# cbs228/sameold

Measured on AMD Instinct MI355X. Metric: Msamples/s demodulated (batched 22.05 kHz channels) + % HBM roofline, 1/8 GPU, higher is better.
Workload: dtype f32

## Files before the change

### include/same_rx.h

```cpp
#ifndef SAME_RX_H
#define SAME_RX_H

#include <stddef.h>
#include <stdint.h>

#ifdef __cplusplus
extern "C" {
#endif

#define SAME_RX_ABI_VERSION 2

enum {
    SAME_OK = 0,
    SAME_EINVAL = -1,
    SAME_EDCLEN = -2,
    SAME_EAGCLIMITS = -3,
    SAME_EEQORDER = -4,
    SAME_ENODEVICE = -5,
    SAME_EHIP = -6,
    SAME_EOVERFLOW = -7,
    SAME_ENOMEM = -8,
    SAME_ERATE = -9,
    SAME_EKERNEL = -10
};
// ... 54 lines not shown

#define SAME_EVENT_MAX_BYTES 288

typedef struct same_rx_event {
    uint32_t kind;
    uint32_t channel;
    uint64_t sample_counter;
    uint64_t symbol_count;
    uint32_t len;
    uint32_t aux;
    uint32_t aux2;
    uint32_t reserved;
    uint8_t bytes[SAME_EVENT_MAX_BYTES];
} same_rx_event;

enum { SAME_LAYOUT_TIME_MAJOR = 0, SAME_LAYOUT_CHANNEL_MAJOR = 1 };

enum {
    SAME_BATCH_LINK_ONLY = 1u << 0,
    SAME_BATCH_TRACE_SYMBOLS = 1u << 1,
    SAME_BATCH_GENERIC_KERNEL = 1u << 2,
    SAME_BATCH_TIME_PARALLEL = 1u << 3,
    SAME_BATCH_RELAXED = 1u << 4,
    SAME_BATCH_CALL_INVARIANT = 1u << 5,
    SAME_BATCH_MESSAGES_ONLY = 1u << 6
};
#define SAME_TP_EVENT_TOLERANCE_SYMBOLS 2

typedef struct same_batch same_batch;

int same_batch_new(const same_rx_builder *b, uint32_t n_channels, int device,
                   uint32_t flags, same_batch **out);
void same_batch_free(same_batch *rx);
int same_batch_reset(same_batch *rx);
int same_batch_reset_channels(same_batch *rx, const uint32_t *channels, size_t n);
uint64_t same_batch_channel_input_sample_counter(const same_batch *rx, uint32_t channel);
uint32_t same_batch_input_rate(const same_batch *rx);
uint32_t same_batch_n_channels(const same_batch *rx);
uint64_t same_batch_input_sample_counter(const same_batch *rx);
int same_batch_device(const same_batch *rx);

#define SAME_STREAM_OWN ((void *)(intptr_t)-1)
int same_batch_process_device(same_batch *rx, const float *d_x, size_t n_samples,
                              uint32_t layout, void *hip_stream);
int same_batch_set_call_window(same_batch *rx, uint32_t samples);
int same_batch_order_after(same_batch *rx, void *producer_stream);
int same_batch_process_device_i16(same_batch *rx, const int16_t *d_x, size_t n_samples,
                                  uint32_t layout, void *hip_stream);
int same_batch_process_host(same_batch *rx, const float *h_x, size_t n_samples, uint32_t layout);
int same_batch_process_host_i16(same_batch *rx, const int16_t *h_x, size_t n_samples, uint32_t layout);
int same_batch_process_device_ragged(same_batch *rx, const float *d_x, size_t n_rows, const uint32_t *counts,
                                     uint32_t layout, void *hip_stream);
int same_batch_process_device_ragged_i16(same_batch *rx, const int16_t *d_x, size_t n_rows, const uint32_t *counts,
                                         uint32_t layout, void *hip_stream);
int same_batch_process_host_ragged(same_batch *rx, const float *h_x, size_t n_rows, const uint32_t *counts, uint32_t layout);
int same_batch_process_host_ragged_i16(same_batch *rx, const int16_t *h_x, size_t n_rows, const uint32_t *counts,
                                       uint32_t layout);
int same_batch_flush(same_batch *rx);
int same_batch_sync(same_batch *rx);

int same_batch_poll_events(same_batch *rx, same_rx_event *out, size_t cap, size_t *n_out,
                           size_t *n_left);
size_t same_batch_pending_events(same_batch *rx);
int same_batch_peek_events(same_batch *rx, const same_rx_event **events, size_t *n);
int same_batch_drop_events(same_batch *rx, size_t n);
#define SAME_BURST_RECORD_BYTES 304
int same_batch_pack_bursts(same_batch *rx, uint32_t first_channel, uint8_t *out, size_t cap, size_t *n_records);

int same_batch_time_parallel_config(same_batch *rx, uint32_t max_chunks, uint32_t min_own_samples,
                                    uint32_t warmup_samples);
uint32_t same_batch_time_parallel_chunks(const same_batch *rx);
int same_batch_time_parallel_per_channel(const same_batch *rx);

typedef struct same_tp_plan_info {
    uint32_t channels, n_chunks, block_len, warmup_samples, whole_samples, scout_blocks;
    uint32_t sort_mode, lpt, pair_groups;
    uint32_t reserved;
    uint64_t in_samples;
    uint64_t counter0;
    uint64_t w_own_start, w_row0, w_nominal, w_perm, w_wg, w_wg2, w_perm2, w_total;
} same_tp_plan_info;
int same_batch_debug_tp_plan(same_batch *rx, same_tp_plan_info *info, float *energy, size_t energy_cap, uint32_t *geom,
                             size_t geom_cap, uint64_t *handover, size_t handover_cap, uint32_t *final_col, size_t final_col_cap);

int same_batch_transport_on_device(const same_batch *rx);

enum {
    SAME_AUDIO_FIRST = 1,
    SAME_AUDIO_END_MESSAGE = 2,
    SAME_AUDIO_END_FLUSH = 4,
    SAME_AUDIO_END_RESET = 8,
    SAME_AUDIO_TRUNCATED = 16
};
typedef struct same_audio_chunk {
    uint32_t channel, flags;
    uint64_t sample_counter;
    uint64_t n_samples;
    const float *samples;
} same_audio_chunk;
int same_batch_set_audio_capture(same_batch *rx, size_t samples_per_launch);
int same_batch_peek_audio(same_batch *rx, const same_audio_chunk **chunks, size_t *n);
int same_batch_drop_audio(same_batch *rx, size_t n);

typedef struct same_symbol_trace {
    uint64_t sample_counter;
    float zero, sym, err, samples_until_next_ted;
} same_symbol_trace;
int same_batch_read_trace(same_batch *rx, uint32_t channel, same_symbol_trace *out,
                          size_t cap, size_t *n_out);

int same_batch_last_kernel_ms(same_batch *rx, float *ms);
int same_batch_last_demod_kernel_ms(same_batch *rx, float *ms);
void same_batch_set_kernel_timing(same_batch *rx, int enable);
const char *same_batch_kernel_name(const same_batch *rx);

typedef struct same_rx same_rx;
int same_rx_build(const same_rx_builder *b, int device, same_rx **out);
void same_rx_free(same_rx *rx);
int same_rx_process(same_rx *rx, const float *x, size_t n, size_t *consumed, same_rx_event *ev);
int same_rx_flush(same_rx *rx, same_rx_event *msg);
int same_rx_reset(same_rx *rx);
uint32_t same_rx_input_rate(const same_rx *rx);
uint64_t same_rx_input_sample_counter(const same_rx *rx);

int same_synth_afsk_device(float *d_x, uint32_t n_channels, size_t n_samples,
                           uint32_t input_rate, uint64_t seed, float noise_sigma,
                           uint32_t flags, int device, void *hip_stream);
uint32_t same_synth_payload(uint64_t seed, uint32_t channel, uint8_t *out, uint32_t cap);
int same_synth_trials_device(float *d_x, uint32_t n_trials, uint32_t first_trial, size_t n_samples,
                             uint32_t input_rate, uint64_t seed, float ebn0_db_lo, float ebn0_db_step,
                             uint32_t n_grid, int device, void *hip_stream);

#ifdef __cplusplus
}
#endif
#endif
```

### sameold_amd/csrc/same_batch.cpp

```cpp
#include <hip/hip_runtime.h>

#include <algorithm>
#include <chrono>
#include <cstdio>
#include <cstdlib>
#include <cstring>
#include <deque>
#include <new>
#include <string>
#include <type_traits>
#include <utility>
#include <vector>

#include "../../include/same_rx.h"
#include "same_config.h"
#include "same_device.h"
#include "same_harvest.h"
#include "same_hipmem.h"
#include "same_launch.h"
#include "same_resets.h"
#include "same_tp_plan.h"
#include "same_transport.h"

using same::fail;
static_assert(sizeof(same::cap::Span) == same::kSpanBytes, "same_tp_plan.h sizes the span list");

namespace {

#define HIP_TRY(expr)                                                                     \
    do {                                                                                   \
        hipError_t _e = (expr);                                                            \
        if (_e != hipSuccess)                                                              \
            return fail(SAME_EHIP, "%s failed: %s (%s:%d)", #expr, hipGetErrorString(_e),  \
                        __FILE__, __LINE__);                                               \
    } while (0)

}

struct same_batch {
    same_rx_builder builder{};
    same::Params P{};
    same::State S{};
    int device = 0;
    uint32_t flags = 0;
    uint64_t counter = 0;
    hipStream_t own_stream = nullptr;
    hipStream_t last_stream = nullptr;
    same::DevBuf<float4> d_taps;
    same::DevBuf<void> d_state_blob;
    struct Slot {
        same::DevBuf<same::DevEvent> d_events;
        uint32_t event_cap() const { return (uint32_t)d_events.size(); }
        same::DevBuf<uint32_t> d_sort;
        same::PinnedBuf<uint32_t> h_sort;
        same::DevBuf<same::DevEvent> d_sorted;
        uint32_t sort_bins = 0;
        same::DevBuf<uint8_t> d_bursts;
        uint32_t burst_cap() const { return (uint32_t)(d_bursts.size() / same::kBurstCap); }
        same::DevBuf<uint32_t> d_counters;
        same::MappedBuf<uint32_t> h_counters;
        same::Event ev_start, ev_stop, ev_done, ev_planned;
        same::Event ev_k0, ev_k1;
        bool have_k = false;
        bool timed = false;
        same::PinnedBuf<void> h_events, h_bursts;
        bool in_flight = false;
        uint64_t seq = 0;
        uint64_t end_counter = 0;
        bool chunked = false;
        same::ChunkGeom geom{};
        uint32_t columns(uint32_t n_channels) const { return chunked ? geom.n_chunks * n_channels : n_channels; }
        uint64_t end_blocks = 0;
        same::DevBuf<uint64_t> d_handover;
        same::PinnedBuf<uint64_t> h_handover;
        bool per_channel = false;
        same::TpGeomWords words;
        same::DevBuf<uint32_t> d_geom;
        same::PinnedBuf<uint32_t> h_geom;
        same::TpPlan plan{};
        uint64_t plan_counter0 = 0;
        bool plan_sorted = false, plan_lpt = false, plan_pairs = false;
        same::CoherentBuf<uint32_t> h_reset;
        same::CoherentBuf<uint32_t> h_counts;
        same::PinnedBuf<uint64_t> h_wake_up;
        bool dev_transport = false;
        same::CoherentBuf<same::DevMessage> h_near;
        uint32_t near_cap() const { return (uint32_t)h_near.size(); }
        same::DevBuf<same::DevMessage> d_msgs;
        uint32_t msg_cap() const { return (uint32_t)d_msgs.size(); }
        same::PinnedBuf<void> h_msgs;
        bool captured = false;
        same::DevBuf<same::cap::Span> d_spans;
        uint32_t span_cap() const { return (uint32_t)d_spans.size(); }
        same::DevBuf<float> d_pool;
        same::DevBuf<same::cap::Cursors> d_cap_cur;
        same::MappedBuf<same::cap::Cursors> h_cap_cur;
        same::PinnedBuf<void> h_spans, h_pool;
    } slot[2];
    struct TimePar {
        bool enabled = false;
        same::TpConfig cfg;
        uint32_t cap_columns = 0;
        uint32_t carved_columns = 0;
        int carved_family = -1;
        same::Params Pv{};
        same::State Sv{};
        same::DevBuf<void> blob;
        same::DevBuf<void> blob_fresh;
        size_t fresh_bytes = 0;
        same::DevBuf<same::StateArrayDesc> d_desc_in, d_desc_out;
        uint32_t n_desc = 0;
        same::DevBuf<uint32_t> d_final_col;
        same::DevBuf<float> d_energy;
        same::DevBuf<float> d_hist;
        same::Event ev_plan_prev; bool plan_recorded = false;
        uint32_t last_chunks = 1;
        bool last_per_channel = false;
        same::Family family = same::Family::kPipe;
    } tp;
    uint64_t launch_seq = 0;
    hipStream_t copy_stream = nullptr;
    struct Windowed {
        bool on = false;
        uint32_t window = 0;
        uint32_t fill = 0;
        same::DevBuf<void> d_buf;
        same::Event ev_buf;
        hipStream_t buf_stream = nullptr; bool buf_used = false;
        same::Event ev_read[2];
        uint64_t n_reads = 0;
        hipStream_t read_stream = nullptr;
    } inv;
    hipStream_t plan_stream = nullptr;
    float last_ms = 0.0f;
    bool overflowed = false;
    std::string record_path;
    bool kernel_fault = false;
    same::Request want;
    same::Mode mode;
    same::Choice plain;
    same::Params Pfm{};
    same::Family last_family = same::Family::kGeneric;
    bool sym_launched = false;
    bool debug = false;
    same::DevBuf<void> d_stage, d_stage2;
    same::DevBuf<void> d_upload;
    same::DevBuf<void> d_zero;
    same::Event ev_order;
    bool timing = false;
    bool have_timing = false;
    float last_demod_ms = 0.0f;
    same::PinnedBuf<uint64_t> h_wake;
    bool wake_ordered = false;
    std::vector<uint32_t> ragged_by;
    bool messages_only = false;
    bool dev_transport = false;
    bool last_dev_transport = false;
    same::DevBuf<void> d_thot, d_tcold;
    same::ResetLedger resets;
    std::vector<uint32_t> reset_list, reset_now, reset_cols;
    same::EventLog events;
    same::Replay replay{resets, events};
    struct Audio {
        size_t per_launch = 0;
        same::DevBuf<same::cap::Rec> d_rec;
        uint64_t flush_at = UINT64_MAX;
        same::AudioLog log;
    } audio;
};

namespace {

struct Carver {
    size_t off = 0;
    template <typename T> size_t take(size_t n)
    {
        off = (off + 255) & ~size_t(255);
        size_t o = off;
        off += n * sizeof(T);
        return o;
    }
};

#define SAME_STATE_ARRAYS(X, P)                                                                            \
    X(dc_ff_ring, float, (P).dc_len) X(dc_fb_ring, float, (P).dc_len)                                        \
    X(dc_sum0, float, 1) X(dc_sum1, float, 1) X(agc_gain, float, 1)                                          \
    X(win_ring, float, (P).win_ring)                                                                         \
    X(ted_clock, uint32_t, 1) X(until_next_ted, float, 1)                                                    \
    X(ted_h0, float, 1) X(ted_h1, float, 1) X(ted_h2, float, 1)                                              \
    X(period_avg, float, 1) X(period_inst, float, 1)                                                         \
    X(sq_data, uint32_t, 1) X(sq_power, float, 1) X(sq_phist, uint32_t, 1)                                   \
    X(sq_fill, uint32_t, 1) X(sq_clock, int32_t, 1) X(sq_symbols, uint64_t, 1)                               \
    X(sq_hist, float, same::kSquelchHist)                                                                    \
    X(eq_ffc, float, (P).eq_nff) X(eq_fbc, float, (P).eq_nfb)                                                \
    X(eq_ffw, float, (P).eq_nff) X(eq_fbw, float, (P).eq_nfb)                                                \
    X(eq_word, uint32_t, 1) X(eq_count, uint32_t, 1)                                                         \
    X(eq_snap_ffc, float, (P).eq_nff) X(eq_snap_fbc, float, (P).eq_nfb)                                      \
// ... 297 lines not shown
    }
    return SAME_OK;
}

int harvest(same_batch *rx)
{
    same_batch::Slot *order[2] = {&rx->slot[0], &rx->slot[1]};
    if (order[0]->seq > order[1]->seq) std::swap(order[0], order[1]);
    for (same_batch::Slot *sl : order) {
        int rc = harvest_slot(rx, *sl);
        if (rc) return rc;
    }
    return SAME_OK;
}

int ensure_wide_state(same_batch *rx, uint32_t columns)
{
    same_batch::TimePar &tp = rx->tp;
    if (tp.carved_columns == columns && tp.carved_family == (int)tp.family) return SAME_OK;
    int rc = harvest(rx);
    if (rc) return rc;
    HIP_TRY(hipDeviceSynchronize());
    tp.Pv = same::wide_params(rx->P, columns, same::is_fastmath(tp.family), same::tp_more_than_one_round(columns));
    if (columns > tp.cap_columns) {
        tp.cap_columns = 0;
        HIP_TRY(tp.blob.reset());
        HIP_TRY(tp.blob_fresh.reset());
        const size_t bytes = carve_state(tp.Pv, nullptr, tp.Sv);
        HIP_TRY(tp.blob.ensure(bytes));
        HIP_TRY(hipMemset(tp.blob, 0, bytes));
        HIP_TRY(tp.blob_fresh.ensure(bytes));
        tp.cap_columns = columns;
    }
    const size_t blob_bytes = carve_state(tp.Pv, (char *)tp.blob.get(), tp.Sv);
    {
        same::State Sf{};
        carve_state(tp.Pv, (char *)tp.blob_fresh.get(), Sf);
        HIP_TRY(hipMemset(tp.blob_fresh, 0, blob_bytes));
        HIP_TRY(same::launch_init_state(tp.Pv, Sf, 0, nullptr, 0));
        HIP_TRY(hipDeviceSynchronize());
        tp.fresh_bytes = (size_t)(reinterpret_cast<char *>(tp.Sv.fr_msg) - static_cast<char *>(tp.blob.get()));
    }
    std::vector<same::StateArrayDesc> in, out;
    list_state_arrays(rx->P, rx->S, tp.Sv, in);
    list_state_arrays(rx->P, tp.Sv, rx->S, out);
    tp.n_desc = (uint32_t)in.size();
    HIP_TRY(tp.d_desc_in.ensure(in.size()));
    HIP_TRY(tp.d_desc_out.ensure(out.size()));
    HIP_TRY(tp.d_final_col.ensure(rx->P.n_channels));
    HIP_TRY(hipMemcpy(tp.d_desc_in, in.data(), in.size() * sizeof(same::StateArrayDesc), hipMemcpyHostToDevice));
    HIP_TRY(hipMemcpy(tp.d_desc_out, out.data(), out.size() * sizeof(same::StateArrayDesc), hipMemcpyHostToDevice));
    tp.carved_columns = columns;
    tp.carved_family = (int)tp.family;
    return SAME_OK;
}

struct Ragged {
    const uint32_t *counts = nullptr;
    uint32_t m = 0;
    uint32_t row_off = 0;
};

struct RaggedLaunch {
    uint32_t row0 = 0;
    size_t n_lock = 0;
};


int begin_launch(same_batch *rx, same_batch::Slot &sl, const same_batch::Slot &prev, hipStream_t stream)
{
    int rc = harvest_slot(rx, sl);
    if (rc) return rc;
    if (prev.in_flight && rx->last_stream != stream) HIP_TRY(hipStreamWaitEvent(stream, prev.ev_done, 0));
    return launch_pending_resets(rx, sl, stream);
}

int begin_timing(same_batch *rx, same_batch::Slot &sl, hipStream_t stream)
{
    sl.timed = rx->timing;
    if (sl.timed) HIP_TRY(hipEventRecord(sl.ev_start, stream));
    return SAME_OK;
}

int tp_start(same_batch *rx, same_batch::Slot &sl, uint32_t columns, const char *layout, hipStream_t stream, bool *sort_bins_empty)
{
    same_batch::TimePar &tp = rx->tp;
    const uint32_t C = rx->P.n_channels;
    *sort_bins_empty = false;
    if (tp.cfg.knob_prologue >= 0) {
        HIP_TRY(same::launch_tp_prologue(tp.blob, tp.blob_fresh, tp.fresh_bytes, sl.d_handover, sl.d_sort, columns, sl.d_counters, stream));
        *sort_bins_empty = sl.sort_bins == columns;
    } else {
        HIP_TRY(same::launch_counters(sl.d_counters, sl.h_counters.dev(), 0, stream));
        HIP_TRY(same::launch_init_state(tp.Pv, tp.Sv, 0, stream, C));
        HIP_TRY(same::launch_fill_u64(sl.d_handover, columns, same::kNoHandover, stream));
    }
    if (rx->debug) std::fprintf(stderr, "[same] time-parallel launch: %u columns (%s), start-up: %s\n", columns, layout,
                                tp.cfg.knob_prologue >= 0 ? "prologue kernel" : "separate launches");
    HIP_TRY(same::launch_copy_state_columns(tp.d_desc_in, tp.n_desc, C, columns, nullptr, C, stream));
    return SAME_OK;
}

template <typename SampleT>
int demod_tail(same_batch *rx, const same::Output &O, const SampleT *rows, size_t n, uint64_t counter0, hipStream_t stream)
{
    const hipError_t e = same::launch_demod(rx->P, rx->S, O, rx->d_taps, rows, (uint32_t)n, counter0, stream);
    if (e != hipSuccess) return fail(SAME_EHIP, "demod kernel launch failed: %s", hipGetErrorString(e));
    return SAME_OK;
}
int demod_tail_corner(same_batch *rx, const same::Output &O, const float *corner, size_t pitch, size_t r, uint64_t counter0, hipStream_t stream)
{
    const uint32_t C = rx->P.n_channels;
    HIP_TRY(rx->d_stage.ensure(r * C * sizeof(float)));
    HIP_TRY(rx->d_stage2.ensure(r * C * sizeof(float)));
    float *staged = static_cast<float *>(rx->d_stage.get()), *rows = static_cast<float *>(rx->d_stage2.get());
    HIP_TRY(hipMemcpy2DAsync(staged, r * sizeof(float), corner, pitch * sizeof(float), r * sizeof(float), C, hipMemcpyDeviceToDevice, stream));
    const hipError_t e = same::launch_transpose(staged, rows, C, (uint32_t)r, stream);
    if (e != hipSuccess) return fail(SAME_EHIP, "demod kernel launch failed: %s", hipGetErrorString(e));
    return demod_tail(rx, O, rows, r, counter0, stream);
}

int tp_plan_boundaries(same_batch *rx, same_batch::Slot &sl, const same::TpCut &cut, const same::TpNative &np, const float *d_x,
                       hipStream_t stream, same::PipeChunks &pc)
{
    same_batch::TimePar &tp = rx->tp;
    const same::TpGeomWords &w = np.words;
    same::TpPlan plan{};
    plan.channels = rx->P.n_channels; plan.n_chunks = cut.n_chunks; plan.block_len = cut.geom.block_len;
    plan.warmup_samples = np.warmup_samples; plan.whole_samples = np.whole_samples; plan.in_samples = np.in_samples;
    plan.scout_blocks = np.scout_blocks;
    sl.plan = plan; sl.plan_counter0 = rx->counter;
    sl.plan_sorted = np.sort_mode != 0; sl.plan_lpt = np.lpt; sl.plan_pairs = np.pair_groups;
    uint32_t *g = sl.d_geom;
    const bool side = same::tp_plan_beside(tp.cfg, stream == rx->own_stream);
    hipStream_t ps = side ? rx->plan_stream : stream;
    if (tp.plan_recorded) HIP_TRY(hipStreamWaitEvent(ps, tp.ev_plan_prev, 0));
    HIP_TRY(same::launch_tp_plan(d_x, plan, tp.d_energy, g + w.own_start, g + w.row0, g + w.nominal, g + w.perm, g + w.wg, np.sort_mode != 0, ps,
                                 np.lpt ? g + w.perm2 : nullptr, np.lpt ? g + w.wg2 : nullptr, np.pair_groups));
    HIP_TRY(tp.ev_plan_prev.ensure());
    HIP_TRY(hipEventRecord(tp.ev_plan_prev, ps));
    tp.plan_recorded = true;
    if (side) {
        HIP_TRY(hipEventRecord(sl.ev_planned, ps));
        HIP_TRY(hipStreamWaitEvent(stream, sl.ev_planned, 0));
    }
    pc.col_row0 = g + w.row0; pc.col_nominal = g + w.nominal;
    pc.wg_blocks = g + (np.lpt ? w.wg2 : w.wg); pc.col_perm = np.lpt ? g + w.perm2 : nullptr;
    pc.in_samples = np.in_samples; pc.whole_samples = np.whole_samples;
    pc.hist_scratch = np.need_hist ? tp.d_hist.get() : nullptr;
    return SAME_OK;
}

template <typename SampleT>
int launch_time_parallel(same_batch *rx, same_batch::Slot &sl, hipStream_t stream, const same::TpCut &cut, const same::TpNative *np,
                         const SampleT *x, size_t n_call, bool *sort_bins_empty)
{
    same_batch::TimePar &tp = rx->tp;
    const same::ChunkGeom &geom = cut.geom;
    const uint32_t C = rx->P.n_channels, columns = cut.n_chunks * C, fb = geom.block_len;
    const uint32_t total_blocks = (uint32_t)(n_call / fb);
    const size_t n_whole = (size_t)total_blocks * fb;
    tp.family = cut.choice.family;
    same::Output O{};
    int rc = ensure_wide_state(rx, columns);
    if (rc == SAME_OK) rc = ensure_output(rx, sl, same::tp_output_samples(np ? n_whole : n_call, cut.pc, fb), O, columns);
    if (rc) return rc;
    HIP_TRY(sl.d_handover.ensure(columns));
    HIP_TRY(sl.h_handover.ensure(columns));
    same::PipeChunks pc = cut.pc;
    pc.handover = sl.d_handover;
    if (np) {
        HIP_TRY(sl.d_geom.ensure(np->words.total));
        HIP_TRY(sl.h_geom.ensure(np->words.harvest));
        HIP_TRY(tp.d_energy.ensure(np->energy_floats));
        if (np->need_hist) HIP_TRY(tp.d_hist.ensure(np->hist_floats));
        sl.words = np->words;
    }
    rc = begin_timing(rx, sl, stream);
    if (rc) return rc;
    const float *xf = nullptr;
    if constexpr (std::is_same_v<SampleT, float>) xf = x;
    if (np && (rc = tp_plan_boundaries(rx, sl, cut, *np, xf, stream, pc)) != SAME_OK) return rc;
    rc = tp_start(rx, sl, columns, np ? "channel-major" : "time-major", stream, sort_bins_empty);
    if (rc) return rc;
    sl.have_k = np && sl.timed;
    if (sl.have_k) HIP_TRY(hipEventRecord(sl.ev_k0, stream));
    const hipError_t e = launch_family(tp.family, tp.Pv, tp.Sv, O, rx->d_taps, x, total_blocks, rx->counter, stream, pc);
    rx->last_family = tp.family;
    if (e != hipSuccess) return fail(SAME_EHIP, "time-parallel demod kernel launch failed: %s", hipGetErrorString(e));
    if (sl.have_k) HIP_TRY(hipEventRecord(sl.ev_k1, stream));
    if (np) HIP_TRY(same::launch_chunk_final_column_pc(sl.d_handover, sl.d_geom + np->words.own_start, C, geom.n_chunks, rx->counter, tp.d_final_col, stream));
    else HIP_TRY(same::launch_chunk_final_column(sl.d_handover, C, geom, tp.d_final_col, stream));
    HIP_TRY(same::launch_copy_state_columns(tp.d_desc_out, tp.n_desc, columns, C, tp.d_final_col, C, stream));
    if (n_whole < n_call) {
        rc = np ? demod_tail_corner(rx, O, xf + n_whole, n_call, n_call - n_whole, rx->counter + n_whole, stream)
                : demod_tail(rx, O, x + n_whole * C, n_call - n_whole, rx->counter + n_whole, stream);
        if (rc) return rc;
    }
    sl.chunked = true; sl.per_channel = np != nullptr;
    sl.geom = geom;
    sl.end_blocks = rx->counter + n_whole;
    tp.last_chunks = cut.n_chunks; tp.last_per_channel = sl.per_channel;
    return SAME_OK;
}

template <typename SampleT>
int end_launch(same_batch *rx, same_batch::Slot &sl, same_batch::Slot &prev, hipStream_t stream, const SampleT *rows, size_t n,
               bool sort_bins_empty, const RaggedLaunch *rl = nullptr)
{
    if (sl.timed) HIP_TRY(hipEventRecord(sl.ev_stop, stream));
    HIP_TRY(same::launch_event_sort(sl.d_events, sl.d_counters, sl.event_cap(), sl.sort_bins, sl.d_sort, sl.d_sort + sl.sort_bins,
                                    sl.d_sorted, stream, sort_bins_empty));
    sl.dev_transport = rx->dev_transport && !sl.chunked;
    rx->last_dev_transport = sl.dev_transport;
    if (sl.dev_transport) {
        same::TransportLaunch T{};
        T.n_channels = rx->P.n_channels; T.input_rate = rx->P.input_rate;
        T.first = sl.d_sort + sl.sort_bins; T.sorted = sl.d_sorted; T.counters = sl.d_counters;
        T.bursts = sl.d_bursts; T.burst_cap = sl.burst_cap();
        T.hot = rx->d_thot; T.cold = rx->d_tcold; T.wake_sample = rx->S.wake_sample;
        T.near = sl.h_near.dev(); T.near_cap = sl.near_cap();
        T.log = sl.d_msgs; T.log_cap = sl.msg_cap(); T.log_cursor = sl.d_counters + 3; T.overflow = sl.d_counters + 2;
        sl.captured = rx->audio.per_launch != 0;
        if (sl.captured) {
            same::cap::Launch &K = T.cap;
            const uint64_t fa = rx->audio.flush_at;
            K.start = rx->counter; K.n_rows = (uint32_t)n;
            K.flush_row = fa >= rx->counter + n ? same::cap::kNoFlush : (uint32_t)(fa > rx->counter ? fa - rx->counter : 0);
            K.rec = rx->audio.d_rec; K.spans = sl.d_spans; K.span_cap = sl.span_cap();
            K.n_spans = &sl.d_cap_cur->n_spans; K.pool_used = &sl.d_cap_cur->pool_used; K.pool_cap = rx->audio.per_launch;
            K.overflow = &sl.d_cap_cur->overflow;
        }
        if (rl && rl->n_lock < n)
            HIP_TRY(same::launch_transport_ragged(T, sl.h_counts.dev(), rl->row0, (uint32_t)n, stream));
        else
            HIP_TRY(same::launch_transport(T, stream));
        if (sl.captured) {
            const hipError_t e = same::launch_capture(sl.d_spans, sl.d_cap_cur, sl.span_cap(), sl.d_pool, rx->audio.per_launch, rows,
                                                      rx->P.n_channels, (uint32_t)n, sl.h_cap_cur.dev(), stream);
            if (e != hipSuccess) return fail(SAME_EHIP, "capture kernel launch failed: %s", hipGetErrorString(e));
        }
    }
    HIP_TRY(same::launch_counters(sl.d_counters, sl.h_counters.dev(), 1, stream));
    HIP_TRY(hipEventRecord(sl.ev_done, stream));
    sl.in_flight = true;
    sl.seq = ++rx->launch_seq;
    rx->last_stream = stream;
    if (rl) rx->resets.shift(rx->ragged_by.data(), rx->counter + n, (int)(&sl - rx->slot));
    rx->counter += n;
    sl.end_counter = rx->counter;
    return harvest_slot(rx, prev);
}

template <typename SampleT>
int process_time_major_launches(same_batch *rx, const SampleT *d_x, size_t n_samples, hipStream_t stream, const Ragged *rg = nullptr)
{
    const size_t kMaxChunk = same::max_launch_samples(rx->P.input_rate);
    size_t done = 0;
    while (done < n_samples) {
        const size_t n = std::min(kMaxChunk, n_samples - done);
        same_batch::Slot &sl = rx->slot[rx->launch_seq & 1];
        same_batch::Slot &prev = rx->slot[(rx->launch_seq & 1) ^ 1];
        int rc = begin_launch(rx, sl, prev, stream);
        if (rc) return rc;
        size_t n_lock = n;
        if (rg) {
            const size_t row0 = (size_t)rg->row_off + done;
            const uint32_t C = rx->P.n_channels;
            HIP_TRY(sl.h_counts.ensure(C));
            std::memcpy(sl.h_counts, rg->counts, (size_t)C * sizeof(uint32_t));
            rx->ragged_by.resize(C);
            n_lock = same::ragged_launch_split(rg->counts, C, rg->m, row0, n, rx->ragged_by.data());
        }
        const same::TpCut cut = rg ? same::TpCut{} : same::tp_uniform_cut(rx->P, rx->mode, rx->want, rx->tp.cfg, n, rx->counter);
        rx->tp.last_chunks = cut.n_chunks;
        sl.have_k = false;
// ... 649 lines not shown
    if (!rx || !n_out) return fail(SAME_EINVAL, "null argument");
    if (!rx->P.trace_cap) return fail(SAME_EINVAL, "batch was not created with SAME_BATCH_TRACE_SYMBOLS");
    if (channel >= rx->P.n_channels) return fail(SAME_EINVAL, "channel out of range");
    HIP_TRY(hipSetDevice(rx->device));
    int rc = harvest(rx);
    if (rc) return rc;
    uint32_t n = 0;
    HIP_TRY(hipMemcpy(&n, rx->S.trace_n + channel, sizeof(n), hipMemcpyDeviceToHost));
    n = std::min(n, rx->P.trace_cap);
    n = (uint32_t)std::min<size_t>(n, cap);
    std::vector<float> f((size_t)n * 4);
    std::vector<uint64_t> idx(n);
    if (n) {
        HIP_TRY(hipMemcpy(f.data(), rx->S.trace + (size_t)channel * rx->P.trace_cap * 4, f.size() * sizeof(float), hipMemcpyDeviceToHost));
        HIP_TRY(hipMemcpy(idx.data(), rx->S.trace_idx + (size_t)channel * rx->P.trace_cap, n * sizeof(uint64_t), hipMemcpyDeviceToHost));
    }
    for (uint32_t i = 0; i < n; ++i) {
        out[i].sample_counter = idx[i];
        out[i].zero = f[4 * i]; out[i].sym = f[4 * i + 1]; out[i].err = f[4 * i + 2];
        out[i].samples_until_next_ted = f[4 * i + 3];
    }
    *n_out = n;
    return SAME_OK;
}

void same_batch_set_kernel_timing(same_batch *rx, int enable) { if (rx) { rx->timing = enable != 0; rx->have_timing = false; } }
int same_batch_last_kernel_ms(same_batch *rx, float *ms)
{
    if (!rx || !ms) return fail(SAME_EINVAL, "null argument");
    if (!rx->have_timing) return fail(SAME_EINVAL, "no timed launch yet");
    *ms = rx->last_ms;
    return SAME_OK;
}
int same_batch_last_demod_kernel_ms(same_batch *rx, float *ms)
{
    if (!rx || !ms) return fail(SAME_EINVAL, "null argument");
    if (!rx->have_timing) return fail(SAME_EINVAL, "no timed launch yet");
    *ms = rx->last_demod_ms;
    return SAME_OK;
}
int same_batch_time_parallel_config(same_batch *rx, uint32_t max_chunks, uint32_t min_own_samples, uint32_t warmup_samples)
{
    if (!rx) return fail(SAME_EINVAL, "null handle");
    if (!rx->tp.enabled) return fail(SAME_EINVAL, "batch was not created with SAME_BATCH_TIME_PARALLEL");
    rx->tp.cfg.max_chunks = max_chunks; rx->tp.cfg.min_own = min_own_samples; rx->tp.cfg.warmup = warmup_samples;
    return SAME_OK;
}
uint32_t same_batch_time_parallel_chunks(const same_batch *rx) { return rx ? rx->tp.last_chunks : 0; }
int same_batch_transport_on_device(const same_batch *rx) { return rx && rx->last_dev_transport ? 1 : 0; }
int same_batch_time_parallel_per_channel(const same_batch *rx) { return rx && rx->tp.last_chunks > 1u && rx->tp.last_per_channel ? 1 : 0; }

int same_batch_debug_tp_plan(same_batch *rx, same_tp_plan_info *info, float *energy, size_t energy_cap, uint32_t *geom,
                             size_t geom_cap, uint64_t *handover, size_t handover_cap, uint32_t *final_col, size_t final_col_cap)
{
    if (!rx || !info) return fail(SAME_EINVAL, "null argument");
    if (rx->launch_seq == 0) return fail(SAME_EINVAL, "no launch yet");
    const same_batch::Slot &sl = rx->slot[(rx->launch_seq - 1) & 1];
    if (!sl.chunked || !sl.per_channel) return fail(SAME_EINVAL, "the last launch had no per-channel plan");
    if (rx->slot[0].in_flight || rx->slot[1].in_flight) return fail(SAME_EINVAL, "a launch is in flight: same_batch_sync first");
    const same::TpPlan &p = sl.plan;
    const same::TpGeomWords &w = sl.words;
    const size_t columns = (size_t)p.n_chunks * p.channels, n_energy = (size_t)p.channels * p.scout_blocks;
    *info = same_tp_plan_info{};
    info->channels = p.channels; info->n_chunks = p.n_chunks; info->block_len = p.block_len;
    info->warmup_samples = p.warmup_samples; info->whole_samples = p.whole_samples; info->scout_blocks = p.scout_blocks;
    info->sort_mode = sl.plan_sorted ? 1u : 0u; info->lpt = sl.plan_lpt ? 1u : 0u; info->pair_groups = sl.plan_pairs ? 1u : 0u;
    info->in_samples = p.in_samples; info->counter0 = sl.plan_counter0;
    info->w_own_start = w.own_start; info->w_row0 = w.row0; info->w_nominal = w.nominal; info->w_perm = w.perm;
    info->w_wg = w.wg; info->w_wg2 = w.wg2; info->w_perm2 = w.perm2; info->w_total = w.total;
    if ((energy && energy_cap < n_energy) || (geom && geom_cap < w.total) || (handover && handover_cap < columns) ||
        (final_col && final_col_cap < p.channels))
        return fail(SAME_EINVAL, "a read-back buffer is too small");
    if (w.total > sl.d_geom.size() || columns > sl.d_handover.size() || n_energy > rx->tp.d_energy.size() ||
        p.channels > rx->tp.d_final_col.size())
        return fail(SAME_EINVAL, "the plan's buffers are gone");
    HIP_TRY(hipSetDevice(rx->device));
    if (energy) HIP_TRY(hipMemcpy(energy, rx->tp.d_energy, n_energy * sizeof(float), hipMemcpyDeviceToHost));
    if (geom) HIP_TRY(hipMemcpy(geom, sl.d_geom, w.total * sizeof(uint32_t), hipMemcpyDeviceToHost));
    if (handover) HIP_TRY(hipMemcpy(handover, sl.d_handover, columns * sizeof(uint64_t), hipMemcpyDeviceToHost));
    if (final_col) HIP_TRY(hipMemcpy(final_col, rx->tp.d_final_col, (size_t)p.channels * sizeof(uint32_t), hipMemcpyDeviceToHost));
    return SAME_OK;
}

const char *same_batch_kernel_name(const same_batch *rx)
{
    return rx ? same::family_name(rx->last_family, rx->P.block_len) : "";
}

}


struct same_rx {
    same_batch *batch = nullptr;
    uint64_t reported = 0;
    uint64_t zeros_until = 0;
    std::deque<same_rx_event> events;
};

static int rx_pump(same_rx *rx)
{
    same_rx_event buf[64];
    for (;;) {
        size_t n = 0, left = 0;
        int rc = same_batch_poll_events(rx->batch, buf, 64, &n, &left);
        if (rc) return rc;
        for (size_t i = 0; i < n; ++i) rx->events.push_back(buf[i]);
        if (!left) return SAME_OK;
    }
}

extern "C" {

int same_rx_build(const same_rx_builder *b, int device, same_rx **out)
{
    if (!out) return fail(SAME_EINVAL, "null out");
    *out = nullptr;
    same_rx *rx = new (std::nothrow) same_rx;
    if (!rx) return fail(SAME_ENOMEM, "out of memory");
    int rc = same_batch_new(b, 1, device, 0, &rx->batch);
    if (rc) { delete rx; return rc; }
    *out = rx;
    return SAME_OK;
}
void same_rx_free(same_rx *rx) { if (rx) { same_batch_free(rx->batch); delete rx; } }

static int rx_process(same_rx *rx, const float *x, size_t n, size_t *consumed, same_rx_event *ev);

int same_rx_process(same_rx *rx, const float *x, size_t n, size_t *consumed, same_rx_event *ev)
{
    if (!rx || !consumed || !ev || (!x && n)) return fail(SAME_EINVAL, "null argument");
    *consumed = 0;
    if (rx->zeros_until > rx->reported && n)
        return fail(SAME_EINVAL, "a flush returned at its first message with the device %llu zero samples ahead; "
                                 "reset the receiver (or flush again) before presenting audio",
                    (unsigned long long)(rx->zeros_until - rx->reported));
    return rx_process(rx, x, n, consumed, ev);
}

static int rx_process(same_rx *rx, const float *x, size_t n, size_t *consumed, same_rx_event *ev)
{
    *consumed = 0;
    const uint64_t device_at = same_batch_input_sample_counter(rx->batch);
    const uint64_t end = rx->reported + n;
    if (end > device_at) {
        const size_t skip = (size_t)(device_at - rx->reported);
        int rc = same_batch_process_host(rx->batch, x + skip, n - skip, SAME_LAYOUT_TIME_MAJOR);
        if (rc) return rc;
        rc = rx_pump(rx);
        if (rc) return rc;
    }
    if (!rx->events.empty() && rx->events.front().sample_counter <= end) {
        *ev = rx->events.front();
        rx->events.pop_front();
        const uint64_t at = ev->sample_counter > rx->reported ? ev->sample_counter : rx->reported;
        *consumed = (size_t)(at - rx->reported);
        rx->reported = at;
        return 1;
    }
    *consumed = n;
    rx->reported = end;
    return 0;
}

int same_rx_flush(same_rx *rx, same_rx_event *msg)
{
    if (!rx) return fail(SAME_EINVAL, "null handle");
// ... 61 lines not shown
```

### sameold_amd/csrc/same_device.h

```cpp
#pragma once

#include <stddef.h>
#include <stdint.h>

namespace same {

constexpr int kWave = 64;
constexpr int kMaxEqTaps = 16;
constexpr int kBurstCap = 288;
constexpr int kSquelchHist = 64;
constexpr int kMaxTaps = 512;

struct Params {
    uint32_t n_channels;
    uint32_t input_rate;
    uint32_t dc_len;
    float dc_inv_len;
    float dc_k;
    float agc_bw, agc_min, agc_max, agc_gain0;
    uint32_t ntaps;
    uint32_t win_ring;
    float samples_per_ted, period_min, period_max;
    float alpha_unlocked, beta_unlocked, alpha_locked, beta_locked;
    uint32_t sync_word, sq_max_errors;
    float sq_power_open, sq_power_close, sq_bw;
    uint32_t eq_nff, eq_nfb;
    float eq_relaxation, eq_regularization;
    uint32_t fr_max_prefix_errors, fr_max_invalid;
    uint32_t block_len;
    uint32_t trace_cap;
    uint32_t ticks;
    uint32_t tick_interburst;
    uint32_t tick_history;
    int32_t knob_pipe;
    int32_t knob_pipe_lanes;
    int32_t knob_pipe_split;
    int32_t knob_mirror;
    int32_t knob_fast_dense;
    int32_t knob_pipe_share;
    int32_t knob_relaxed_kernel;
    int32_t knob_sym;
    int32_t knob_prio;
};

enum : uint32_t {
    F_AGC_LOCKED = 1u << 0,
    F_TED_PHASE = 1u << 1,
    F_BW_LOCKED = 1u << 2,
    F_SQ_LOCK = 1u << 3,
    F_EQ_MODE_SHIFT = 4,
    F_EQ_MODE_MASK = 3u << 4,
    F_FR_STATE_SHIFT = 6,
    F_FR_STATE_MASK = 3u << 6,
    F_LINK_SHIFT = 8,
    F_LINK_MASK = 3u << 8,
    F_TICK_AGAIN = 1u << 10,
    F_EQ_BITS_SHIFT = 16,
    F_EQ_BITS_MASK = 0xffu << 16,
};
constexpr int kTickRing = 8;

struct State {
    float *dc_ff_ring;
    float *dc_fb_ring;
    float *dc_sum0, *dc_sum1;
    float *agc_gain;
    float *win_ring;
    uint32_t *ted_clock;
    float *until_next_ted;
    float *ted_h0, *ted_h1, *ted_h2;
    float *period_avg, *period_inst;
    uint32_t *sq_data;
    float *sq_power;
    uint32_t *sq_phist;
    uint32_t *sq_fill;
    int32_t *sq_clock;
    uint64_t *sq_symbols;
    float *sq_hist;
    float *eq_ffc, *eq_fbc;
    float *eq_ffw, *eq_fbw;
    uint32_t *eq_word, *eq_count;
    float *eq_snap_ffc, *eq_snap_fbc, *eq_snap_ffw, *eq_snap_fbw;
    uint32_t *fr_word, *fr_count, *fr_invalid, *fr_len;
    uint8_t *fr_msg;
    uint32_t *flags;
    uint64_t *tk_next;
    uint64_t *tk_last;
    uint64_t *tk_ring;
    uint32_t *tk_n;
    uint64_t *wake_sample;
    uint64_t *wake_fired;
    uint32_t *trace_n;
    float *trace;
    uint64_t *trace_idx;
};

struct PipeChunks {
    uint32_t n_chunks;
    uint32_t in_channels;
    uint32_t stride_blocks;
    uint32_t nominal_blocks;
    uint64_t *handover;
    const uint32_t *col_row0;
    const uint32_t *col_nominal;
    const uint32_t *wg_blocks;
    const uint32_t *col_perm;
    float *hist_scratch;
    uint64_t in_samples;
    uint32_t whole_samples;
};

struct ChunkGeom {
    uint64_t counter0;
    uint32_t n_chunks, block_len, stride_blocks, warmup_blocks;
#if defined(__HIPCC__)
    __host__ __device__
#endif
    uint32_t owner_of(uint64_t h) const
    {
        const uint64_t blocks = (h - counter0) / block_len;
        if (blocks < warmup_blocks) return 0u;
        const uint64_t k = (blocks - warmup_blocks) / stride_blocks;
        return k >= n_chunks ? n_chunks - 1u : (uint32_t)k;
    }
#if defined(__HIPCC__)
    __host__ __device__
#endif
    uint64_t own_start(uint32_t k) const
    { return k == 0u ? counter0 : counter0 + ((uint64_t)k * stride_blocks + warmup_blocks) * block_len; }
};
constexpr uint64_t kNoHandover = ~0ull;

struct StateArrayDesc { char *src; char *dst; uint32_t rows; uint32_t elem_words; };

constexpr uint32_t kDevEventNone = 0xffffffffu;
struct DevEvent {
    uint32_t channel;
    uint32_t kind;
    uint64_t sample_counter;
    uint64_t symbol_count;
    uint32_t burst_len;
    uint32_t burst_slot;
};

constexpr uint32_t kDevMessageText = 272;
struct DevMessage {
    uint32_t channel;
    uint32_t kind;
    uint64_t sample_counter;
    uint64_t symbol_count;
    uint32_t len, aux, aux2;
    uint32_t seq;
    uint8_t text[kDevMessageText];
};

struct Output {
    DevEvent *events;
    uint32_t *n_events;
    uint32_t event_cap;
    uint8_t *bursts;
    uint32_t *n_bursts;
    uint32_t burst_cap;
    uint32_t *overflow;
};

}
```

### sameold_amd/csrc/same_kernels.hip

```cpp
#include <hip/hip_runtime.h>

#include <algorithm>

#include "same_dev_common.h"
#include "same_device.h"
#include "same_launch.h"
#include "same_tp_plan.h"

namespace same {

template <int B, typename SampleT>
__global__ __launch_bounds__(kWave) void demod_kernel(Params P, State S, Output O,
                                                      const float4 *__restrict__ taps,
                                                      const SampleT *__restrict__ x,
                                                      uint32_t n_samples, uint64_t counter0)
{
    extern __shared__ float lds[];
    const uint32_t lane = threadIdx.x;
    const uint32_t C = P.n_channels;
    const uint32_t c_raw = blockIdx.x * kWave + lane;
    if (c_raw >= C) return;
    const uint32_t c = c_raw;
    const uint32_t DL = P.dc_len;
    float *ff = lds;
// ... 345 lines not shown
    hipLaunchKernelGGL(ev_hist_kernel, dim3(256), dim3(256), 0, stream, ev, counters, cap, n_bins, cnt);
    const uint32_t scan_grid = (n_bins + kScanThreads - 1u) / kScanThreads;
    uint32_t *tot = first + n_bins + 1u;
    hipLaunchKernelGGL(ev_scan_local_kernel, dim3(scan_grid), dim3(kScanThreads), 0, stream, n_bins, cnt, first, tot);
    hipLaunchKernelGGL(ev_scan_base_kernel, dim3(scan_grid), dim3(kScanThreads), 0, stream, n_bins, cnt, first, tot);
    hipLaunchKernelGGL(ev_scatter_kernel, dim3(256), dim3(256), 0, stream, ev, counters, cap, n_bins, cnt, sorted);
    return hipGetLastError();
}

template <typename SampleT>
static hipError_t launch_demod_t(const Params &P, const State &S, const Output &O, const float4 *taps,
                                 const SampleT *x, uint32_t n_samples, uint64_t counter0,
                                 hipStream_t stream)
{
    const uint32_t grid = (P.n_channels + kWave - 1) / kWave;
    const size_t lds = (size_t)(2 * P.dc_len + P.win_ring) * kWave * sizeof(float);
#define SAME_LAUNCH(BV)                                                                          \
    hipLaunchKernelGGL((demod_kernel<BV, SampleT>), dim3(grid), dim3(kWave), lds, stream, P, S, \
                       O, taps, x, n_samples, counter0)
    switch (P.block_len) {
    case 16: SAME_LAUNCH(16); break;
    case 8: SAME_LAUNCH(8); break;
    case 4: SAME_LAUNCH(4); break;
    case 2: SAME_LAUNCH(2); break;
    default: SAME_LAUNCH(1); break;
    }
#undef SAME_LAUNCH
    return hipGetLastError();
}

hipError_t launch_demod(const Params &P, const State &S, const Output &O, const float4 *taps,
                        const float *x, uint32_t n_samples, uint64_t counter0, hipStream_t stream)
{ return launch_demod_t<float>(P, S, O, taps, x, n_samples, counter0, stream); }

hipError_t launch_demod(const Params &P, const State &S, const Output &O, const float4 *taps,
                        const int16_t *x, uint32_t n_samples, uint64_t counter0, hipStream_t stream)
{ return launch_demod_t<int16_t>(P, S, O, taps, x, n_samples, counter0, stream); }

template <typename SampleT>
static hipError_t launch_demod_ragged_t(const Params &P, const State &S, const Output &O, const float4 *taps, const SampleT *x,
                                        uint32_t n_rows, const uint32_t *counts, uint32_t row_sub, uint64_t counter0,
                                        hipStream_t stream)
{
    const uint32_t grid = (P.n_channels + kWave - 1) / kWave;
    const size_t lds = (size_t)(2 * P.dc_len + P.win_ring) * kWave * sizeof(float);
#define SAME_LAUNCH(BV)                                                                                 \
    hipLaunchKernelGGL((demod_ragged_kernel<BV, SampleT>), dim3(grid), dim3(kWave), lds, stream, P, S, \
                       O, taps, x, n_rows, counts, row_sub, counter0)
    switch (P.block_len) {
    case 16: SAME_LAUNCH(16); break;
    case 8: SAME_LAUNCH(8); break;
    case 4: SAME_LAUNCH(4); break;
    case 2: SAME_LAUNCH(2); break;
    default: SAME_LAUNCH(1); break;
    }
#undef SAME_LAUNCH
    return hipGetLastError();
}

hipError_t launch_demod_ragged(const Params &P, const State &S, const Output &O, const float4 *taps, const float *x,
                               uint32_t n_rows, const uint32_t *counts, uint32_t row_sub, uint64_t counter0, hipStream_t stream)
{ return launch_demod_ragged_t<float>(P, S, O, taps, x, n_rows, counts, row_sub, counter0, stream); }

hipError_t launch_demod_ragged(const Params &P, const State &S, const Output &O, const float4 *taps, const int16_t *x,
                               uint32_t n_rows, const uint32_t *counts, uint32_t row_sub, uint64_t counter0, hipStream_t stream)
{ return launch_demod_ragged_t<int16_t>(P, S, O, taps, x, n_rows, counts, row_sub, counter0, stream); }

hipError_t launch_init_state(const Params &P, const State &S, int is_reset, hipStream_t stream, uint32_t first_col)
{
    if (first_col >= P.n_channels) return hipSuccess;
    const uint32_t grid = (P.n_channels - first_col + 255) / 256;
    hipLaunchKernelGGL(init_state_kernel, dim3(grid), dim3(256), 0, stream, P, S, is_reset, first_col);
    return hipGetLastError();
}

hipError_t launch_reset_columns(const Params &P, const State &S, const uint32_t *cols, uint32_t n, hipStream_t stream)
{
    if (!n) return hipSuccess;
    hipLaunchKernelGGL(reset_columns_kernel, dim3((n + 63u) / 64u), dim3(64), 0, stream, P, S, cols, n);
    return hipGetLastError();
}

__global__ void copy_state_columns_kernel(const StateArrayDesc *desc, uint32_t Csrc, uint32_t Cdst,
                                          const uint32_t *src_col, uint32_t n_cols, uint32_t src_base)
{
    const uint32_t col = blockIdx.x * blockDim.x + threadIdx.x;
    if (col >= n_cols) return;
    const StateArrayDesc d = desc[blockIdx.y];
    const uint32_t sc = src_col ? src_col[col] : col + src_base;
    const uint32_t w = d.elem_words;
    const uint32_t *src = reinterpret_cast<const uint32_t *>(d.src);
    uint32_t *dst = reinterpret_cast<uint32_t *>(d.dst);
    const uint32_t n = d.rows * w;
    for (uint32_t k = blockIdx.z; k < n; k += gridDim.z) {
        const uint32_t r = k / w, i = k - r * w;
        dst[((size_t)r * Cdst + col) * w + i] = src[((size_t)r * Csrc + sc) * w + i];
    }
}
hipError_t launch_copy_state_columns(const StateArrayDesc *desc, uint32_t n_desc, uint32_t src_channels,
                                     uint32_t dst_channels, const uint32_t *src_col, uint32_t n_cols, hipStream_t stream,
                                     uint32_t src_base)
{
    hipLaunchKernelGGL(copy_state_columns_kernel, dim3((n_cols + 255) / 256, n_desc, 16), dim3(256), 0, stream, desc,
                       src_channels, dst_channels, src_col, n_cols, src_base);
    return hipGetLastError();
}
__global__ void chunk_final_column_kernel(const uint64_t *handover, uint32_t C, ChunkGeom g, uint32_t *final_col)
{
    const uint32_t c = blockIdx.x * blockDim.x + threadIdx.x;
    if (c >= C) return;
    uint32_t cur = 0;
    for (;;) {
        const uint64_t h = handover[(size_t)cur * C + c];
        if (h == kNoHandover) break;
        const uint32_t nxt = g.owner_of(h);
        if (nxt <= cur) break;
        cur = nxt;
    }
    final_col[c] = cur * C + c;
}
hipError_t launch_chunk_final_column(const uint64_t *handover, uint32_t in_channels, ChunkGeom g, uint32_t *final_col,
                                     hipStream_t stream)
{
    hipLaunchKernelGGL(chunk_final_column_kernel, dim3((in_channels + 255) / 256), dim3(256), 0, stream, handover, in_channels, g, final_col);
    return hipGetLastError();
}
__global__ void chunk_final_column_pc_kernel(const uint64_t *handover, const uint32_t *own_start, uint32_t C, uint32_t K,
                                             uint64_t counter0, uint32_t *final_col)
{
    const uint32_t c = blockIdx.x * blockDim.x + threadIdx.x;
    if (c >= C) return;
    uint32_t cur = 0;
    for (;;) {
        const uint64_t h = handover[(size_t)cur * C + c];
        if (h == kNoHandover) break;
        uint32_t nxt = cur;
        for (uint32_t k = cur + 1u; k < K; ++k)
            if (counter0 + own_start[(size_t)k * C + c] <= h) nxt = k;
        if (nxt <= cur) break;
        cur = nxt;
    }
    final_col[c] = cur * C + c;
}
hipError_t launch_chunk_final_column_pc(const uint64_t *handover, const uint32_t *own_start, uint32_t in_channels, uint32_t n_chunks,
                                        uint64_t counter0, uint32_t *final_col, hipStream_t stream)
{
    hipLaunchKernelGGL(chunk_final_column_pc_kernel, dim3((in_channels + 255) / 256), dim3(256), 0, stream, handover, own_start,
                       in_channels, n_chunks, counter0, final_col);
    return hipGetLastError();
}
__global__ void tp_scout_kernel(const float *__restrict__ x, TpPlan g, float *__restrict__ energy)
{
    const size_t t = (size_t)blockIdx.x * blockDim.x + threadIdx.x;
    const size_t i = t >> 2;
    const uint32_t q = (uint32_t)t & 3u;
    const bool live = i < (size_t)g.channels * g.scout_blocks;
    float e = 0.0f;
    if (live) {
        const uint32_t c = (uint32_t)(i / g.scout_blocks), j = (uint32_t)(i % g.scout_blocks);
        const float4 v = reinterpret_cast<const float4 *>(x + (size_t)c * g.in_samples + (size_t)j * kScoutBlock)[q];
        e = (fabsf(v.x) + fabsf(v.y)) + (fabsf(v.z) + fabsf(v.w));
    }
    e += __shfl_xor(e, 1);
    e += __shfl_xor(e, 2);
    if (live && q == 0u) energy[i] = e;
}
__global__ __launch_bounds__(kWave) void tp_boundaries_kernel(const float *__restrict__ energy, TpPlan g, uint32_t *__restrict__ own_start,
                                                               uint32_t *__restrict__ row0, uint32_t *__restrict__ nominal)
{
    extern __shared__ float tp_lds[];
    const uint32_t c = blockIdx.x, lane = threadIdx.x;
    const int NB = (int)g.scout_blocks, K = (int)g.n_chunks;
    float *e = tp_lds;
    int *lastq = reinterpret_cast<int *>(tp_lds + NB);
    int *cut = lastq + NB;
    constexpr int kQuietBefore = 2048 / (int)kScoutBlock, kQuietAfter = 1;
    float m = 0.0f;
    for (int j = (int)lane; j < NB; j += (int)kWave) { const float v = energy[(size_t)c * NB + j]; e[j] = v; m = fmaxf(m, v); }
    for (int off = 32; off > 0; off >>= 1) m = fmaxf(m, __shfl_xor(m, off));
    const float thr = 0.08f * m;
    __syncthreads();
    const int S = (NB + (int)kWave - 1) / (int)kWave, j0 = (int)lane * S, j1 = min(j0 + S, NB);
    int run = -1;
    for (int j = j0; j < j1; ++j) {
        bool ok = j - kQuietBefore >= 0 && j + kQuietAfter < NB;
        if (ok) for (int t = j - kQuietBefore; t <= j + kQuietAfter; ++t) if (e[t] > thr) { ok = false; break; }
        if (ok) run = j;
// ... 52 lines not shown
}
constexpr uint32_t kSortBuckets = 4096, kSortBucketBlocks = 4;
__device__ __forceinline__ void tp_sort_key(const TpPlan &g, const uint32_t *row0, const uint32_t *nominal, uint32_t v,
                                            uint32_t *group, uint32_t *bucket)
{
    const uint32_t chunk = v / g.channels;
    const uint32_t avail = (g.whole_samples - row0[v]) / g.block_len;
    *group = chunk + 1u == g.n_chunks ? 0u : (chunk == 0u ? 1u : 2u);
    const uint32_t len = *group == 0u ? avail : min(nominal[v], avail);
    *bucket = kSortBuckets - 1u - min(len / kSortBucketBlocks, kSortBuckets - 1u);
}
constexpr uint32_t kSortThreads = 1024;
__global__ __launch_bounds__(kSortThreads) void tp_sort_kernel(TpPlan g, const uint32_t *__restrict__ row0, const uint32_t *__restrict__ nominal,
                                                                uint32_t *__restrict__ perm)
{
    __shared__ uint32_t hist[3u * kSortBuckets];
    __shared__ uint32_t wave_sum[kSortThreads / kWave];
    const uint32_t tid = threadIdx.x, lane = tid & (kWave - 1u), wave = tid / kWave, n = g.n_chunks * g.channels;
    for (uint32_t i = tid; i < 3u * kSortBuckets; i += kSortThreads) hist[i] = 0u;
    __syncthreads();
    for (uint32_t v = tid; v < n; v += kSortThreads) {
        uint32_t grp, b;
        tp_sort_key(g, row0, nominal, v, &grp, &b);
        if (grp != 0u) atomicAdd(&hist[grp * kSortBuckets + b], 1u);
    }
    __syncthreads();
    constexpr uint32_t PER = kSortBuckets / kSortThreads;
    static_assert(PER * kSortThreads == kSortBuckets, "buckets per thread");
    const uint32_t base[3] = {0u, g.channels, 2u * g.channels};
    for (uint32_t grp = 0; grp < 3u; ++grp) {
        uint32_t *h = hist + grp * kSortBuckets + tid * PER;
        uint32_t mine = 0;
        for (uint32_t i = 0; i < PER; ++i) mine += h[i];
        uint32_t incl = mine;
        for (int off = 1; off < (int)kWave; off <<= 1) { const uint32_t t = (uint32_t)__shfl_up((int)incl, off); if ((int)lane >= off) incl += t; }
        if (lane == kWave - 1u) wave_sum[wave] = incl;
        __syncthreads();
        uint32_t before = base[grp] + incl - mine;
        for (uint32_t w = 0; w < wave; ++w) before += wave_sum[w];
        for (uint32_t i = 0; i < PER; ++i) { const uint32_t c = h[i]; h[i] = before; before += c; }
        __syncthreads();
    }
    for (uint32_t v = tid; v < n; v += kSortThreads) {
        uint32_t grp, b;
        tp_sort_key(g, row0, nominal, v, &grp, &b);
        if (grp == 0u) perm[v - (g.n_chunks - 1u) * g.channels] = v;
        else perm[atomicAdd(&hist[grp * kSortBuckets + b], 1u)] = v;
    }
}
__global__ void tp_iota_kernel(uint32_t *perm, uint32_t n)
{
    const uint32_t i = blockIdx.x * blockDim.x + threadIdx.x;
    if (i < n) perm[i] = i;
}
__global__ void tp_align_kernel(TpPlan g, const uint32_t *__restrict__ perm, uint32_t *__restrict__ row0, const uint32_t *__restrict__ nominal,
                                uint32_t *__restrict__ wg_blocks, uint32_t *__restrict__ wg_len)
{
    const uint32_t v = perm[blockIdx.x * kWave + threadIdx.x];
    const uint32_t chunk = v / g.channels;
    uint32_t avail = (g.whole_samples - row0[v]) / g.block_len;
    uint32_t m = avail;
    for (int off = 32; off > 0; off >>= 1) m = max(m, (uint32_t)__shfl_xor((int)m, off));
    if (chunk + 1u == g.n_chunks) row0[v] = g.whole_samples - m * g.block_len;
    if (threadIdx.x == 0) wg_blocks[blockIdx.x] = m;
    if (wg_len) {
        uint32_t len = chunk + 1u == g.n_chunks ? m : min(nominal[v], avail);
        for (int off = 32; off > 0; off >>= 1) len = max(len, (uint32_t)__shfl_xor((int)len, off));
        if (threadIdx.x == 0) wg_len[blockIdx.x] = len;
    }
}
__global__ void tp_wg_order_kernel(uint32_t n_wg, const uint32_t *__restrict__ perm, const uint32_t *__restrict__ wg_blocks,
                                   const uint32_t *__restrict__ wg_len, uint32_t *__restrict__ perm_out, uint32_t *__restrict__ wg_blocks_out,
                                   uint32_t pairs)
{
    const uint32_t w = blockIdx.x, lane = threadIdx.x;
    const uint32_t mine = wg_len[w];
    uint32_t rank = 0;
    for (uint32_t j = lane; j < n_wg; j += kWave) { const uint32_t b = wg_len[j]; rank += (b > mine || (b == mine && j < w)) ? 1u : 0u; }
    for (int off = 32; off > 0; off >>= 1) rank += (uint32_t)__shfl_xor((int)rank, off);
    const uint32_t pos = (pairs && (n_wg & 1u) == 0u) ? (rank < n_wg / 2u ? 2u * rank : 2u * (n_wg - 1u - rank) + 1u) : rank;
    perm_out[pos * kWave + lane] = perm[w * kWave + lane];
    if (lane == 0) wg_blocks_out[pos] = wg_blocks[w];
}
hipError_t launch_tp_plan(const float *x, const TpPlan &g, float *energy, uint32_t *own_start, uint32_t *row0,
                          uint32_t *nominal, uint32_t *perm, uint32_t *wg_blocks, bool sorted, hipStream_t stream,
                          uint32_t *perm_out, uint32_t *wg_blocks_out, bool pairs)
{
    const size_t n = (size_t)g.channels * g.scout_blocks;
    const uint32_t columns = g.n_chunks * g.channels;
    hipLaunchKernelGGL(tp_scout_kernel, dim3((unsigned)((4 * n + 255) / 256)), dim3(256), 0, stream, x, g, energy);
    hipLaunchKernelGGL(tp_boundaries_kernel, dim3(g.channels), dim3(kWave), (size_t)g.scout_blocks * 8 + 64 * sizeof(int), stream, energy, g, own_start, row0, nominal);
    if (sorted) {
        hipLaunchKernelGGL(tp_sort_kernel, dim3(1), dim3(kSortThreads), 0, stream, g, row0, nominal, perm);
    } else {
        hipLaunchKernelGGL(tp_iota_kernel, dim3((columns + 255) / 256), dim3(256), 0, stream, perm, columns);
    }
    uint32_t *wg_len = perm_out ? wg_blocks_out + columns / kWave : nullptr;
    hipLaunchKernelGGL(tp_align_kernel, dim3(columns / kWave), dim3(kWave), 0, stream, g, perm, row0, nominal, wg_blocks, wg_len);
    if (perm_out)
        hipLaunchKernelGGL(tp_wg_order_kernel, dim3(columns / kWave), dim3(kWave), 0, stream, columns / kWave, perm, wg_blocks, wg_len,
                           perm_out, wg_blocks_out, pairs ? 1u : 0u);
    return hipGetLastError();
}

__global__ __launch_bounds__(256) void tp_prologue_kernel(uint4 *__restrict__ dst, const uint4 *__restrict__ src, size_t n16,
                                                          uint64_t *__restrict__ handover, uint32_t *__restrict__ sort_cnt, uint32_t n_cols,
                                                          uint32_t *__restrict__ counters)
{
    const size_t t = (size_t)blockIdx.x * blockDim.x + threadIdx.x, stride = (size_t)gridDim.x * blockDim.x;
    for (size_t i = t; i < n16; i += stride) dst[i] = src[i];
    for (size_t i = t; i < n_cols; i += stride) { handover[i] = kNoHandover; if (sort_cnt) sort_cnt[i] = 0u; }
    if (t < 3 && counters) counters[t] = 0u;
}
hipError_t launch_tp_prologue(void *blob, const void *fresh, size_t bytes, uint64_t *handover, uint32_t *sort_cnt, uint32_t n_cols,
                              uint32_t *counters, hipStream_t stream)
{
    const size_t n16 = bytes / 16;
    const unsigned grid = (unsigned)std::min<size_t>((n16 + 255) / 256, 256 * 16);
    hipLaunchKernelGGL(tp_prologue_kernel, dim3(grid ? grid : 1u), dim3(256), 0, stream, reinterpret_cast<uint4 *>(blob),
                       reinterpret_cast<const uint4 *>(fresh), n16, handover, sort_cnt, n_cols, counters);
    return hipGetLastError();
}
__global__ void cast_i16_f32_kernel(const int16_t *__restrict__ in, float *__restrict__ out, size_t n)
{
    for (size_t i = (size_t)blockIdx.x * blockDim.x + threadIdx.x; i < n; i += (size_t)gridDim.x * blockDim.x) out[i] = (float)in[i];
}
hipError_t launch_cast_i16_f32(const int16_t *in, float *out, size_t n, hipStream_t stream)
{
    if (!n) return hipSuccess;
    hipLaunchKernelGGL(cast_i16_f32_kernel, dim3((unsigned)std::min<size_t>((n + 255) / 256, 65536)), dim3(256), 0, stream, in, out, n);
    return hipGetLastError();
}
__global__ void fill_u64_kernel(uint64_t *p, size_t n, uint64_t v)
{
    const size_t i = (size_t)blockIdx.x * blockDim.x + threadIdx.x;
    if (i < n) p[i] = v;
}
hipError_t launch_fill_u64(uint64_t *p, size_t n, uint64_t v, hipStream_t stream)
{
    hipLaunchKernelGGL(fill_u64_kernel, dim3((unsigned)((n + 255) / 256)), dim3(256), 0, stream, p, n, v);
    return hipGetLastError();
}

hipError_t launch_transpose(const float *in, float *out, uint32_t n_channels, uint32_t n_samples,
                            hipStream_t stream)
{
    dim3 grid((n_samples + 63) / 64, (n_channels + 63) / 64);
    hipLaunchKernelGGL(transpose_to_time_major<float>, grid, dim3(256), 0, stream, in, out, n_channels, n_samples);
    return hipGetLastError();
}
hipError_t launch_transpose(const int16_t *in, int16_t *out, uint32_t n_channels, uint32_t n_samples,
                            hipStream_t stream)
{
    dim3 grid((n_samples + 63) / 64, (n_channels + 63) / 64);
    hipLaunchKernelGGL(transpose_to_time_major<int16_t>, grid, dim3(256), 0, stream, in, out, n_channels, n_samples);
    return hipGetLastError();
}

}
```

### sameold_amd/csrc/same_kernels_sym.hip

```cpp
#include <hip/hip_runtime.h>

#include <cmath>
#include <cstdlib>
#include <mutex>
#include <set>
#include <type_traits>
#include <utility>

#include "same_dev_common.h"
#include "same_device.h"
#include "same_fast_common.h"
#include "same_launch.h"
#include "same_pipe_common.h"
#include "same_profile.h"
#include "same_relaxed_common.h"

namespace same {

constexpr int kSymSub = 36;
constexpr uint32_t kSymDrain = 5u;
constexpr uint32_t kSymOffMask = 255u;
template <int NT> struct SymGeom;
template <> struct SymGeom<42> { static constexpr int DCL = 16, NSUB = 1, HALVES = 2; };
template <> struct SymGeom<92> { static constexpr int DCL = 35, NSUB = 2, HALVES = 1; };
// ... 822 lines not shown
    const uint32_t link_ready = restart ? (burst_at_restart ? 3u : 1u) : (over ? 3u : nst);
    const uint32_t link_quiet = reading ? st : (st == 2u ? 3u : 0u);
    const uint32_t link = ready ? link_ready : link_quiet;
    F.st = ready ? nst : ((valid & !reading) ? 0u : st);
    const uint32_t fb_end = FB_VALID | FB_END | (((m >> YM_OFF_SHIFT) & kSymOffMask) << 8);
    *fb2 = ready ? (link == 2u ? (uint32_t)FB_SQLOCK : ((link == 0u || link == 3u) ? fb_end : 0u)) : 0u;
    *emit = valid & ((link != F.last) | (link == 3u));
    F.last = *emit ? link : F.last;
    return link;
}

#ifndef SYM_PRIOS
#define SYM_PRIOS 0x0031322
#endif
constexpr int sym_prio_of(int k) { return (int)((SYM_PRIOS >> (4 * (6 - k))) & 3); }
#ifndef SYM_PRIOS_HI
#define SYM_PRIOS_HI 0x3321200
#endif
template <int NT> constexpr int sym_prio(int k) { return NT == 42 ? sym_prio_of(k) : (int)((SYM_PRIOS_HI >> (4 * (6 - k))) & 3); }
template <int PRIO> __device__ __forceinline__ void sym_setprio(const Params &P)
{
#ifdef SAME_PROFILE
    const uint32_t variant = ((uint32_t)P.knob_prio >> 12) & 3u;
    if (variant == 1u) return;
    if (variant == 2u) { __builtin_amdgcn_s_setprio(PRIO >= 2 ? 3 : 0); return; }
#else
    (void)P;
#endif
    __builtin_amdgcn_s_setprio(PRIO);
}

__device__ __forceinline__ float sym_next_fire(float s)
{
    return fmaxf(floorf(s - 0.5f) + 1.0f, 1.0f);
}

struct SymKernArgs { Params P; State S; Output O; const float4 *taps; const void *x; uint32_t n_blocks; uint64_t counter0; PipeChunks K; };
typedef const __attribute__((address_space(4))) char *sym_kernarg_ptr;
template <typename T> __device__ __forceinline__ T sym_fresh_arg(sym_kernarg_ptr ka, size_t off)
{
    uint64_t p = (uint64_t)(uintptr_t)ka + off;
    asm volatile("" : "+s"(p));
    T r;
    __builtin_memcpy(&r, reinterpret_cast<const __attribute__((address_space(4))) void *>(p), sizeof(T));
    return r;
}

constexpr int kSymRoles = 6;
template <int NT, int NFF, int NFB, typename SampleT, int CMODE>
__global__ __launch_bounds__(SymGeom<NT>::HALVES * kSymRoles * kWave, NT == 42 ? 3 : 2) void demod_sym_kernel(Params P, State S_arg_, Output O_arg_, const float4 *__restrict__ taps,
                                                                         const SampleT *__restrict__ x, uint32_t n_blocks, uint64_t counter0,
                                                                         PipeChunks K)
{
    (void)S_arg_; (void)O_arg_;
    const sym_kernarg_ptr ka = (sym_kernarg_ptr)__builtin_amdgcn_kernarg_segment_ptr();
    auto fresh_state = [&]() __attribute__((always_inline)) -> State { return sym_fresh_arg<State>(ka, offsetof(SymKernArgs, S)); };
    auto fresh_output = [&]() __attribute__((always_inline)) -> Output { return sym_fresh_arg<Output>(ka, offsetof(SymKernArgs, O)); };
    using LY = SymLayout<NT>;
    constexpr int kB = LY::B, RING = LY::RING, kSB = LY::SB, kNSUB = LY::NSUB;
    constexpr uint32_t kSymHalves = (uint32_t)LY::HALVES;
    constexpr uint32_t LP = kWave;
    static_assert(CMODE == 0 || std::is_same<SampleT, float>::value, "channel-major streams are f32");
    if constexpr (CMODE == 0) { K.col_row0 = nullptr; K.col_perm = nullptr; }
    extern __shared__ float lds_all[];
    const uint32_t lane = threadIdx.x & (kWave - 1u);
    const uint32_t wave = (uint32_t)__builtin_amdgcn_readfirstlane((int)(threadIdx.x >> 6));
    constexpr uint64_t kDeal0 = 0xdcba98543210ull;
#ifdef SAME_PROFILE
    const uint32_t deal = ((uint32_t)P.knob_prio >> 14) & 3u;
    constexpr uint64_t kDeal1 = 0x805d192ab3c4ull;
    constexpr uint64_t kDeal2 = 0x08d591a2b3c4ull;
    constexpr uint64_t kDeal3 = 0x2ad51908b3c4ull;
    const uint64_t tbl = deal == 0u ? kDeal0 : (deal == 1u ? kDeal1 : (deal == 2u ? kDeal2 : kDeal3));
#else
    constexpr uint64_t tbl = kDeal0;
#endif
    const uint32_t hr = LY::HALVES == 2 ? (uint32_t)(tbl >> (4u * wave)) & 15u : wave;
    const uint32_t half = LY::HALVES == 2 ? hr >> 3 : 0u;
    const uint32_t role = hr & 7u;
    const uint32_t C = P.n_channels;
    const uint32_t vwg = blockIdx.x * kSymHalves + half;
    if (vwg * kWave >= C) return;
    float *lds = lds_all + half * (uint32_t)(LY::lds_bytes / sizeof(float));
    const uint32_t c = (K.n_chunks > 1u && K.col_perm) ? K.col_perm[vwg * kWave + lane] : vwg * kWave + lane;
    uint32_t cin = c, Cin = C, n_nominal = n_blocks;
    bool may_leave = false;
    int32_t row_l = 0;
    const SampleT *xl = nullptr;
    uint32_t avail_l = 0;
    if (K.n_chunks > 1u) {
        Cin = K.in_channels;
        if (K.col_row0) {
            const uint32_t chunk_l = c / Cin;
            cin = c - chunk_l * Cin;
            may_leave = (uint32_t)__builtin_amdgcn_readfirstlane((int)chunk_l) + 1u < K.n_chunks;
            const uint32_t row_abs = K.col_row0[c];
            xl = x + (size_t)cin * K.in_samples + row_abs;
            avail_l = (K.whole_samples - row_abs) / (uint32_t)kSB;
            n_blocks = K.wg_blocks[vwg];
            n_nominal = may_leave ? K.col_nominal[c] : n_blocks;
            const uint32_t row_first = (uint32_t)__builtin_amdgcn_readfirstlane((int)row_abs);
            counter0 += (uint64_t)row_first;
            row_l = (int32_t)(row_abs - row_first);
        } else {
            const uint32_t wgs = K.in_channels / kWave;
            const uint32_t chunk = (uint32_t)__builtin_amdgcn_readfirstlane((int)(vwg / wgs));
            cin = (vwg - chunk * wgs) * kWave + lane;
            may_leave = chunk + 1u < K.n_chunks;
            const uint32_t first_block = chunk * K.stride_blocks;
            x += (size_t)first_block * kB * Cin;
            counter0 += (uint64_t)first_block * kB;
            n_blocks -= first_block;
            n_nominal = may_leave ? K.nominal_blocks : n_blocks;
        }
    }
    lds_u32 *mail = (lds_u32 *)(lds + LY::tap_floats);
    lds_u32 *symbox = mail;
    lds_u32 *ybox = symbox + 2u * LY::sym_words;
    lds_u32 *fb1box = ybox + 2u * kWave;
    lds_u32 *fb2box = fb1box + 2u * LY::fb_words;
    lds_u32 *iobox = fb2box + 2u * LY::fb_words;
    lds_u32 *phasebox = iobox + 2u * LY::io_words;
    lds_u32 *againbox = phasebox + kWave;
    lds_u32 *flagbox = againbox + kWave;
    lds_u32 *posbox = flagbox + kWave;
    lds_u32 *sabox = posbox + 2u * kWave;
    lds_u32 *tkbox = sabox + kWave;
    lds_u32 *donebox = tkbox + kIoRingWords;
    lds_u32 *chunkbox = fb1box + kWave + 2u;
    lds_u32 *seqbox = fb1box + kWave + 4u;
    static_assert((size_t)(2u * LY::sym_words + 2u * kWave + 4u * LY::fb_words + 2u * LY::io_words + 3u * kWave + 2u * kWave + kWave + kIoRingWords + kWave + kWave) <= LY::mail_words, "mailboxes");
    float *wring = lds + LY::tap_floats + LY::mail_words;
    float *wcol = wring + lane;
    const uint64_t counter1 = counter0 + (uint64_t)n_blocks * kB;
    const uint32_t last_e_step = n_blocks + kSymDrain;
    const uint32_t last_y1_step = last_e_step + 1u, last_y2_step = last_e_step + 2u, last_a_step = last_e_step + 3u;
    const uint32_t n_steps = last_e_step + 4u;
    auto sym_index = [&](uint32_t s_e, uint32_t off) __attribute__((always_inline)) -> int64_t {
        const int64_t base = s_e <= n_blocks ? (int64_t)s_e - 2 : (int64_t)n_blocks - 3;
        return (int64_t)kB * base + (int64_t)off;
    };
    lds_u32 *prog = donebox + kWave;
    lds_u32 *pos2box = prog + kWave + (SYM_TL_WORDS + 63u) / 64u * 64u;
    lds_u32 *partbox = pos2box + 2u * kWave;
#ifdef SAME_SYM_TL
    lds_u32 *tlbox = prog + kWave;
#endif
    const uint32_t prog_idx = lane < (uint32_t)kSymRoles ? lane : 0u;
    uint32_t *const err_flags = fresh_output().n_events + 2;
    uint32_t spin_limit = 1u << 22;
    auto gave_up = [&]() __attribute__((always_inline)) -> bool { return spin_limit != (1u << 22); };
    constexpr bool kPeek = NT != 42;
    uint32_t seen = 0u;
    auto peek = [&]() __attribute__((always_inline)) { if constexpr (kPeek) seen = prog[prog_idx]; };
    auto wait_for = [&](uint32_t s, uint32_t deps, uint32_t *w_y1, uint32_t *w_y2, auto nap_) __attribute__((always_inline)) {
        constexpr int NAP = decltype(nap_)::value;
        uint32_t v = seen, spins = 0;
        if constexpr (!kPeek) v = prog[prog_idx];
        for (;;) {
            const uint32_t ok = (uint32_t)__builtin_amdgcn_ballot_w64(v >= (s << 16));
            if ((ok & deps) == deps) break;
            if (!kPeek || spins != 0u) __builtin_amdgcn_s_sleep(NAP);
            if (++spins > spin_limit) { if (lane == 0u) atomicOr(err_flags, 4u); spin_limit = 8u; break; }
            v = prog[prog_idx];
        }
        if constexpr (kPeek) seen = v;
        asm volatile("" ::: "memory");
        *w_y1 = (uint32_t)__builtin_amdgcn_readlane((int)v, 4);
        *w_y2 = (uint32_t)__builtin_amdgcn_readlane((int)v, 5);
    };
    constexpr std::integral_constant<int, 1> kNapShort{};
    constexpr std::integral_constant<int, 4> kNapLong{};
    auto flags_of_last = [&](uint32_t w, uint32_t s) __attribute__((always_inline)) -> uint32_t { return s == 0u ? 0u : (w >> (8u * ((s - 1u) & 1u))) & 0xffu; };
    auto publish = [&](uint32_t s, uint32_t flags, uint32_t flags_before) __attribute__((always_inline)) {
        asm volatile("" ::: "memory");
        if (lane == 0u) prog[role] = ((s + 1u) << 16) | (flags << (8u * (s & 1u))) | (flags_before << (8u * ((s + 1u) & 1u)));
    };
    enum : uint32_t { R_S = 1u, R_T = 2u, R_A = 4u, R_E = 8u, R_Y1 = 16u, R_Y2 = 32u };
    enum : uint32_t { Y1F_ANY = 1u, Y2F_END = 1u, Y2F_LEAVE = 2u, Y2F_LOCK = 4u };
    constexpr uint32_t kDepsS = R_T | R_A | R_E | R_Y1 | R_Y2;
    if (role == 0u && lane < (uint32_t)kSymRoles) prog[lane] = 0u;

    if (role == 0u) {
        sym_setprio<sym_prio<NT>(0)>(P);
        SymAgc<NT> M;
        { const State S = fresh_state(); M.load(P, S, c, C, counter0, wcol); }
        lds_barrier();
        P3_T0();
        uint32_t stop_at = 0xffffffffu;
        bool left = false;
        for (uint32_t s = 0; s < n_steps; ++s) {
            uint32_t w1, w2;
            SYM_TRACE(0, s, 0);
            wait_for(s, kDepsS, &w1, &w2, kNapLong);
            SYM_TRACE(0, s, 1);
            P3_LAP(p3_wait);
            const uint32_t f1 = flags_of_last(w1, s), f2 = flags_of_last(w2, s);
            if (f2 & Y2F_LEAVE) stop_at = s;
            if ((f2 & Y2F_END) && s >= 1u) {
                if (fb2box[((s - 1u) & 1u) * LY::fb_words + lane] & FB_VALID) M.locked = false;
            }
            if ((f1 & Y1F_ANY) && s >= 1u) {
                const uint32_t v = fb1box[((s - 1u) & 1u) * LY::fb_words + lane];
                if (v & FB_VALID) {
                    const bool new_locked = (v & FB_AGC) != 0u;
                    if (new_locked && !M.locked) {
                        const int64_t idx = sym_index(s - 2u, v >> 8);
                        const uint32_t b = (uint32_t)(idx / kB);
                        M.gain = M.gain_at(P, wcol, b, (int)(idx - (int64_t)b * kB));
                    }
                    M.locked = new_locked;
                }
                P3_LAP(p3_fb);
            }
            if (s < n_blocks && !PROF_SKIP(P, 64)) M.block(P, wcol, s);
            SYM_TRACE(0, s, 2);
            peek();
            publish(s, 0u, 0u);
            P3_LAP(p3_work);
            if (s == stop_at) { left = true; break; }
        }
        SYM_REPORT(0);
        if (left || gave_up()) return;
        { const State S = fresh_state(); M.store(P, S, c, C, counter1, wcol); }
    } else if (role == 1u) {
        sym_setprio<sym_prio<NT>(1)>(P);
        if constexpr (NT != 42) {
            static_assert(CMODE == 0 && kNSUB == 2, "time-major rows, two sub-blocks a step");
            SymDcRot<SampleT, NT> D;
            const uint32_t n_sub = n_blocks * (uint32_t)kNSUB;
            { const State S = fresh_state(); D.load(S, x, c, C, cin, Cin, counter0, n_sub); }
            donebox[lane] = 0u;
            D.template sub<0>(P, wcol, x, 0u, n_sub, cin, Cin);
            D.template sub<1>(P, wcol, x, 1u, n_sub, cin, Cin);
            lds_barrier();
            P3_T0();
            uint32_t stop_at = 0xffffffffu;
            auto step = [&](uint32_t s, auto ph_) __attribute__((always_inline)) -> bool {
                constexpr int PH = 2 * decltype(ph_)::value;
                uint32_t w1, w2;
                SYM_TRACE(1, s, 0);
                wait_for(s, R_A | R_E, &w1, &w2, kNapLong);
                SYM_TRACE(1, s, 1);
                P3_LAP(p3_wait);
                if (s + 1u < n_blocks && !PROF_SKIP(P, 128)) {
                    D.template sub<PH>(P, wcol, x, 2u * (s + 1u), n_sub, cin, Cin);
                    D.template sub<PH + 1>(P, wcol, x, 2u * (s + 1u) + 1u, n_sub, cin, Cin);
                }
                if (may_leave) {
                    wait_for(s, R_Y2, &w1, &w2, kNapLong);
                    if (flags_of_last(w2, s) & Y2F_LEAVE) stop_at = s;
                }
                SYM_TRACE(1, s, 2);
                peek();
                publish(s, 0u, 0u);
                P3_LAP(p3_work);
                return s == stop_at;
            };
            bool left = false;
            for (uint32_t s = 0; s < n_steps && !left; s += 3u) {
                left = step(s, std::integral_constant<int, 1>{});
                if (!left && s + 1u < n_steps) left = step(s + 1u, std::integral_constant<int, 2>{});
                if (!left && s + 2u < n_steps) left = step(s + 2u, std::integral_constant<int, 0>{});
            }
            SYM_REPORT(1);
            if (left || gave_up()) return;
            { const State S = fresh_state(); D.store(S, c, C, counter1, n_sub - 1u); }
            return;
        } else {
        using Dc = SymDc<SampleT, CMODE, NT>;
        Dc D;
        D.xl = xl; D.avail = avail_l;
        const uint32_t n_sub = n_blocks * (uint32_t)kNSUB;
        { const State S = fresh_state(); D.load(S, x, c, C, cin, Cin, counter0, n_sub); }
        donebox[lane] = 0u;
        auto sub_tm = [&](uint32_t q, auto pb_) __attribute__((always_inline)) {
            typename Dc::Pairs X;
            if constexpr (decltype(pb_)::value == 0) { D.request(D.xb, x, q + 1u, n_sub, cin, Cin); D.template take<0>(D.xa, X); }
            else { D.request(D.xa, x, q + 1u, n_sub, cin, Cin); D.template take<0>(D.xb, X); }
            D.block(P, wcol, X, q);
        };
        {
            if constexpr (CMODE == 1) {
                typename Dc::Pairs X0;
                D.request(D.xb, x, 1u, n_sub, cin, Cin);
                D.template take<9>(D.xa, X0);
                D.block(P, wcol, X0, 0u);
                D.request(D.xa, x, 2u, n_sub, cin, Cin);
            } else {
                sub_tm(0u, std::integral_constant<int, 0>{});
                if constexpr (kNSUB == 2) sub_tm(1u, std::integral_constant<int, 1>{});
            }
        }
        lds_barrier();
        P3_T0();
        uint32_t stop_at = 0xffffffffu;
        auto step = [&](uint32_t s, auto buf) __attribute__((always_inline)) -> bool {
            constexpr int BUF = decltype(buf)::value;
            uint32_t w1, w2;
            SYM_TRACE(1, s, 0);
            wait_for(s, R_A | R_E, &w1, &w2, kNapLong);
            SYM_TRACE(1, s, 1);
            P3_LAP(p3_wait);
            if constexpr (CMODE == 1) D.done = donebox[lane] != 0u;
            if (s + 1u < n_blocks && !PROF_SKIP(P, 128)) {
                if constexpr (CMODE == 1) {
                    typename Dc::Pairs X;
                    if constexpr (BUF == 0) { D.template take<9>(D.xa, X); D.block(P, wcol, X, s + 1u); D.request(D.xa, x, s + 3u, n_sub, cin, Cin); }
                    else { D.template take<9>(D.xb, X); D.block(P, wcol, X, s + 1u); D.request(D.xb, x, s + 3u, n_sub, cin, Cin); }
                } else if constexpr (kNSUB == 1) {
                    sub_tm(s + 1u, buf);
                } else {
                    sub_tm(2u * (s + 1u), std::integral_constant<int, 0>{});
                    sub_tm(2u * (s + 1u) + 1u, std::integral_constant<int, 1>{});
                }
            }
            if (may_leave) {
                wait_for(s, R_Y2, &w1, &w2, kNapLong);
                if (flags_of_last(w2, s) & Y2F_LEAVE) stop_at = s;
            }
            SYM_TRACE(1, s, 2);
            peek();
            publish(s, 0u, 0u);
            P3_LAP(p3_work);
            return s == stop_at;
        };
        bool left = false;
        for (uint32_t s = 0; s < n_steps && !left; s += 2u) {
            left = step(s, std::integral_constant<int, 1>{});
            if (!left && s + 1u < n_steps) left = step(s + 1u, std::integral_constant<int, 0>{});
        }
        SYM_REPORT(1);
        if (left || gave_up()) return;
        { const State S = fresh_state(); D.store(S, c, C, counter1); }
        }
    } else if (role == 2u) {
        sym_setprio<sym_prio<NT>(2)>(P);
        const uint32_t wcol_lds = lds_addr(wcol);
        std::conditional_t<NT == 42, SymTaps<42>, SymHalfTaps<NT, 0, NT / 4>> TP;
        TP.load(taps);
        Lane L;
        IoCtxLds X;
        X.chunk = chunkbox;
        if (lane == 0u) { chunkbox[0] = 0u; chunkbox[1] = kEvChunk; seqbox[0] = 0u; }
        X.pending_slot = 0xffffffffu;
        X.tk = tkbox + lane;
        {
            const State S = fresh_state();
            lane_load(L, S, c);
            X.ring_load(P, S, c);
        }
        const State Snone{};
        Output O{};
        { const Output Of = fresh_output(); O.events = Of.events; O.n_events = Of.n_events; O.event_cap = Of.event_cap; }
        lds_barrier();
        P3_T0();
        uint32_t stop_at = 0xffffffffu;
        bool left = false;
        for (uint32_t s = 0; s < n_steps; ++s) {
            uint32_t w1, w2;
            SYM_TRACE(2, s, 0);
            wait_for(s, R_S | R_E, &w1, &w2, kNapShort);
            SYM_TRACE(2, s, 1);
            P3_LAP(p3_wait);
            if (s >= 1u && s <= last_e_step) {
                const uint32_t n1 = posbox[(s & 1u) * kWave + lane];
                if constexpr (NT == 42) {
                    if (__builtin_amdgcn_ballot_w64(n1 != 0xffffffffu) != 0ull) {
                        const float sa1 = PROF_SKIP(P, 256) ? 0.0f : TP.template demod<RING>(wcol_lds, n1 == 0xffffffffu ? 0 : (int)n1);
                        sabox[lane] = __float_as_uint(sa1);
                        if (lane == 0u) seqbox[0] = 2u * s + 1u;
                    }
                } else {
                    const uint32_t n2 = pos2box[(s & 1u) * kWave + lane];
                    if (__builtin_amdgcn_ballot_w64(n2 != 0xffffffffu) != 0ull) {
                        float2v r2 = {0.0f, 0.0f}, i2 = {0.0f, 0.0f}, r1 = {0.0f, 0.0f}, i1 = {0.0f, 0.0f};
                        if (!PROF_SKIP(P, 256)) {
                            TP.template partial<RING>(wcol_lds, n2 == 0xffffffffu ? 0 : (int)n2, r2, i2);
                            if (__builtin_amdgcn_ballot_w64(n1 != 0xffffffffu) != 0ull) TP.template partial<RING>(wcol_lds, n1 == 0xffffffffu ? 0 : (int)n1, r1, i1);
                        }
                        lds_u32 *pb = partbox + lane;
                        pb[0] = __float_as_uint(r2.x); pb[kWave] = __float_as_uint(r2.y); pb[2 * kWave] = __float_as_uint(i2.x); pb[3 * kWave] = __float_as_uint(i2.y);
                        pb[4 * kWave] = __float_as_uint(r1.x); pb[5 * kWave] = __float_as_uint(r1.y); pb[6 * kWave] = __float_as_uint(i1.x); pb[7 * kWave] = __float_as_uint(i1.y);
                        if (lane == 0u) seqbox[0] = 2u * s + 1u;
                    }
                }
            }
            SYM_TRACE(2, s, 3);
            sym_setprio<sym_prio<NT>(3)>(P);
            wait_for(s, R_Y2, &w1, &w2, kNapLong);
            if (flags_of_last(w2, s) & Y2F_LEAVE) stop_at = s;
            if (s >= 4u && s <= last_a_step && !PROF_SKIP(P, 8)) {
                const lds_u32 *io = iobox + ((s - 1u) & 1u) * LY::io_words + lane;
                const uint32_t io0 = io[0];
                if (io0 & 1u) {
                    L.sq_symbols += 1;
                    const uint32_t link = (io0 >> 1) & 3u, off = (io0 >> 4) & kSymOffMask;
                    const bool burst = (io0 & 8u) != 0u && link == 3u;
                    uint32_t burst_len = 0;
                    if (burst) { X.pending_slot = io[kWave]; burst_len = io[2 * kWave]; }
                    const uint64_t counter = counter0 + (int64_t)row_l + (uint64_t)sym_index(s - 3u, off) + 1u;
                    symbol_io(P, L, Snone, O, X, c, link, (io0 & 8u) != 0u, counter, burst_len);
                }
            }
            if (s + 1u == n_steps) againbox[lane] = L.flags & F_TICK_AGAIN;
            SYM_TRACE(2, s, 2);
            peek();
            publish(s, 0u, 0u);
            sym_setprio<sym_prio<NT>(2)>(P);
            P3_LAP(p3_work);
            if (s == stop_at) { left = true; break; }
        }
        SYM_REPORT(2);
        X.retire(O, lane, kWave);
        if (left || gave_up()) return;
        {
            const State S = fresh_state();
            S.tk_next[c] = L.tk_next; S.tk_last[c] = L.tk_last; S.wake_fired[c] = L.wake_fired;
            X.ring_store(P, S, c);
        }
    } else if (role == 3u) {
        sym_setprio<sym_prio<NT>(4)>(P);
        const uint32_t wcol_lds = lds_addr(wcol);
        std::conditional_t<NT == 42, SymTaps<42>, SymHalfTaps<NT, NT / 4, NT / 2>> TP;
        TP.load(taps);
        Lane L;
        { const State S = fresh_state(); lane_load(L, S, c); }
        const float inv_spt = 1.0f / P.samples_per_ted;
        int cstar = next_fire_count(L.until_next_ted, L.ted_clock);
        int rel = cstar - (int)L.ted_clock - 1;
        float cstar_f = (float)cstar;
        SYM_T_DECL();
        bool pl_typeA = false, pl_ready = false, pl_single = false;
        int pl_p2 = 0;
        uint32_t pl_n2 = 0, pl_n1 = 0xffffffffu;
        float pl_rem1 = 0.0f, pl_instA = 0.0f, pl_c2 = 0.0f;
        auto plan = [&](uint32_t s) __attribute__((always_inline)) {
            pl_single = s > n_blocks;
            const uint32_t wb = (min(s, n_blocks) % (uint32_t)LY::NBLK) * (uint32_t)kB;
            pl_typeA = !pl_single && (L.flags & F_TED_PHASE) != 0u;
            pl_rem1 = L.until_next_ted - cstar_f;
            pl_instA = L.period_inst + __builtin_amdgcn_fmed3f(pl_rem1, -0.5f, 0.5f);
            pl_c2 = sym_next_fire(pl_instA);
            pl_p2 = pl_typeA ? rel + (int)pl_c2 : rel;
            pl_ready = pl_p2 < 0 && s >= 1u && s <= last_e_step;
            auto slot = [&](int p) __attribute__((always_inline)) { int n = (int)wb + p; n += n < 0 ? RING : 0; return (uint32_t)n; };
            pl_n2 = pl_ready ? slot(pl_p2) : 0u;
            pl_n1 = (pl_ready && pl_typeA) ? slot(rel) : 0xffffffffu;
            posbox[(s & 1u) * kWave + lane] = pl_n1;
            if constexpr (NT != 42) pos2box[(s & 1u) * kWave + lane] = pl_ready ? pl_n2 : 0xffffffffu;
        };
        float sa1 = 0.0f, sa2 = 0.0f;
        auto filters = [&](uint32_t seq) __attribute__((always_inline)) {
            sa1 = 0.0f; sa2 = 0.0f;
            if (__builtin_amdgcn_ballot_w64(pl_ready) != 0ull) {
                SYM_T_BEGIN();
                SYM_TCOUNT(20, 1);
                auto wait_for_a = [&]() __attribute__((always_inline)) {
                    uint32_t spins = 0;
                    while ((int32_t)(seqbox[0] - seq) < 0) {
                        __builtin_amdgcn_s_sleep(1);
                        if (++spins > spin_limit) { if (lane == 0u) atomicOr(err_flags, 4u); spin_limit = 8u; break; }
                    }
                    asm volatile("" ::: "memory");
                };
                if constexpr (NT == 42) {
                    sa2 = PROF_SKIP(P, 512) ? 0.0f : TP.template demod<RING>(wcol_lds, (int)pl_n2);
                    SYM_T_LAP(22);
                    if (__builtin_amdgcn_ballot_w64(pl_ready && pl_typeA) != 0ull) {
                        wait_for_a();
                        sa1 = __uint_as_float(sabox[lane]);
                    }
                } else {
                    float2v r2 = {0.0f, 0.0f}, i2 = {0.0f, 0.0f}, r1 = {0.0f, 0.0f}, i1 = {0.0f, 0.0f};
                    const bool any_a = __builtin_amdgcn_ballot_w64(pl_n1 != 0xffffffffu) != 0ull;
                    if (!PROF_SKIP(P, 512)) {
                        TP.template partial<RING>(wcol_lds, (int)pl_n2, r2, i2);
                        if (any_a) TP.template partial<RING>(wcol_lds, pl_n1 == 0xffffffffu ? 0 : (int)pl_n1, r1, i1);
                    }
                    SYM_T_LAP(22);
                    wait_for_a();
                    const lds_u32 *pb = partbox + lane;
                    r2 += float2v{__uint_as_float(pb[0]), __uint_as_float(pb[kWave])}; i2 += float2v{__uint_as_float(pb[2 * kWave]), __uint_as_float(pb[3 * kWave])};
                    sa2 = sym_soft_sample(r2, i2);
                    if (any_a) {
                        r1 += float2v{__uint_as_float(pb[4 * kWave]), __uint_as_float(pb[5 * kWave])}; i1 += float2v{__uint_as_float(pb[6 * kWave]), __uint_as_float(pb[7 * kWave])};
                        sa1 = sym_soft_sample(r1, i1);
                    }
                }
                SYM_T_LAP(24);
            }
        };
        auto work = [&](uint32_t s) __attribute__((always_inline)) {
            SYM_T_BEGIN();
            const bool rdy = pl_ready, tA = pl_typeA;
            const float p1 = tA ? L.h2 : L.h1, p2 = tA ? sa1 : L.h2;
            const float inst_pre = tA ? pl_instA : L.period_inst;
            const float rem = tA ? pl_instA - pl_c2 : pl_rem1;
            const uint32_t flags_new = tA ? L.flags : (L.flags ^ F_TED_PHASE);
            const bool have = (flags_new & F_TED_PHASE) != 0u;
            const float dsg = rs_signum(p1) - rs_signum(sa2);
            const float te = p2 * dsg;
            const float offset = __builtin_amdgcn_fmed3f(rem, -0.5f, 0.5f);
            const float e = __builtin_amdgcn_fmed3f(__builtin_fmaf(-offset, inv_spt, te), -1.0f, 1.0f);
            const bool bw_locked = (L.flags & F_BW_LOCKED) != 0u;
            const float alpha = bw_locked ? P.alpha_locked : P.alpha_unlocked;
            const float beta = bw_locked ? P.beta_locked : P.beta_unlocked;
            const float avg1 = __builtin_amdgcn_fmed3f(__builtin_fmaf(beta, e, L.period_avg), P.period_min, P.period_max);
            float inst1 = __builtin_fmaf(alpha, e, avg1) + offset;
            inst1 = (inst1 < 0.0f) ? avg1 : inst1;
            const float inst_new = have ? inst1 : inst_pre + offset;
            const float cs = sym_next_fire(inst_new);
            const bool take = rdy & have;
            L.h0 = rdy ? p1 : L.h0; L.h1 = rdy ? p2 : L.h1; L.h2 = rdy ? sa2 : L.h2;
            L.flags = rdy ? flags_new : L.flags;
            L.period_avg = take ? avg1 : L.period_avg;
            L.period_inst = rdy ? inst_new : L.period_inst; L.until_next_ted = rdy ? inst_new : L.until_next_ted;
            cstar_f = rdy ? cs : cstar_f;
            rel = rdy ? pl_p2 + (int)cs : rel;
            const uint32_t hdr = take ? (1u | ((uint32_t)(pl_p2 + (pl_single ? 3 * kB : 2 * kB)) << 8)) : 0u;
            SYM_T_LAP(23);
            lds_u32 *sb = symbox + (s & 1u) * LY::sym_words + lane;
            sb[0] = hdr;
            sb[kWave] = __float_as_uint(p2); sb[2 * kWave] = __float_as_uint(sa2);
            if (P.trace_cap) { sb[3 * kWave] = __float_as_uint(te); sb[4 * kWave] = __float_as_uint(inst_new); }
        };
        auto late = [&](uint32_t v) __attribute__((always_inline)) {
            if (v & FB_VALID) {
                L.flags = (L.flags & ~F_BW_LOCKED) | ((v & FB_BW) ? F_BW_LOCKED : 0u);
                if (v & FB_END) {
                    L.flags &= ~F_TED_PHASE;
                    L.h0 = 0.0f; L.h1 = 0.0f; L.h2 = 0.0f;
                    L.period_avg = P.samples_per_ted; L.period_inst = P.samples_per_ted;
                }
            }
        };
        plan(0u);
        lds_barrier();
        P3_T0();
        uint32_t stop_at = 0xffffffffu;
        bool left = false;
        for (uint32_t s = 0; s < n_steps; ++s) {
            uint32_t w1, w2;
            SYM_TRACE(3, s, 0);
            wait_for(s, R_S, &w1, &w2, kNapShort);
            SYM_TRACE(3, s, 1);
            P3_LAP(p3_wait);
            if (!PROF_SKIP(P, 32)) filters(2u * s + 1u);
            wait_for(s, R_A | R_Y1 | R_Y2, &w1, &w2, kNapShort);
            SYM_TRACE(3, s, 3);
            const uint32_t f1 = flags_of_last(w1, s), f2 = flags_of_last(w2, s);
            if (f2 & Y2F_LEAVE) stop_at = s;
            uint32_t late1 = 0u, late2 = 0u;
            if ((f1 & Y1F_ANY) && s >= 1u) late1 = fb1box[((s - 1u) & 1u) * LY::fb_words + lane];
            if ((f2 & Y2F_END) && s >= 1u) late2 = fb2box[((s - 1u) & 1u) * LY::fb_words + lane];
            if (!PROF_SKIP(P, 32)) {
                work(s);
                if (__builtin_amdgcn_ballot_w64(((late1 | late2) & FB_VALID) != 0u) != 0ull) { late(late2); late(late1); }
                if (s + 1u <= n_blocks) rel -= kB;
                plan(s + 1u);
            }
            if (s + 1u == n_steps) phasebox[lane] = L.flags & F_TED_PHASE;
            SYM_TRACE(3, s, 2);
            peek();
            publish(s, 0u, 0u);
            P3_LAP(p3_work);
            if (s == stop_at) { left = true; break; }
        }
        SYM_REPORT(3);
        SYM_T_REPORT();
        if (left || gave_up()) return;
        L.ted_clock = (uint32_t)((int)cstar_f - rel - 1);
        {
            const State S = fresh_state();
            S.until_next_ted[c] = L.until_next_ted; S.ted_clock[c] = L.ted_clock;
            S.ted_h0[c] = L.h0; S.ted_h1[c] = L.h1; S.ted_h2[c] = L.h2;
            S.period_avg[c] = L.period_avg; S.period_inst[c] = L.period_inst;
        }
    } else if (role == 4u) {
        sym_setprio<sym_prio<NT>(5)>(P);
        SymSquelch<NFF, NFB> Q;
        uint64_t symbols0;
        const bool hist_copy = K.n_chunks > 1u && K.col_perm != nullptr && K.hist_scratch != nullptr;
        {
            const State S = fresh_state();
            lane_load(Q.L, S, c);
            symbols0 = Q.L.sq_symbols;
            Q.nsym = (uint32_t)symbols0;
            Q.hbase = reinterpret_cast<char *>(hist_copy ? K.hist_scratch : S.sq_hist);
            Q.hcol4 = (hist_copy ? vwg * kWave + lane : c) * 4u;
            Q.hrow4 = C * 4u;
            if (hist_copy) {
#pragma unroll 4
                for (int i = 0; i < kSquelchHist; ++i) *Q.hptr((uint32_t)i) = S.sq_hist[(size_t)i * C + c];
            }
#pragma unroll
            for (int i = 0; i < NFF; ++i) {
                Q.ffc[i] = S.eq_ffc[i * C + c]; Q.ffw[i] = S.eq_ffw[i * C + c];
                Q.sffc[i] = S.eq_snap_ffc[i * C + c]; Q.sffw[i] = S.eq_snap_ffw[i * C + c];
            }
#pragma unroll
            for (int i = 0; i < NFB; ++i) {
                Q.fbc[i] = S.eq_fbc[i * C + c]; Q.fbw[i] = S.eq_fbw[i * C + c];
                Q.sfbc[i] = S.eq_snap_fbc[i * C + c]; Q.sfbw[i] = S.eq_snap_fbw[i * C + c];
            }
            const uint32_t pslot = (2u * Q.nsym) & 63u;
            Q.nxt0 = *Q.hptr((pslot + 16u) & 63u); Q.nxt1 = *Q.hptr((pslot + 17u) & 63u);
        }
        lds_barrier();
        P3_T0();
        uint32_t stop_at = 0xffffffffu, flags_before = 0u, last_msg = 0u;
        bool left = false;
        for (uint32_t s = 0; s < n_steps; ++s) {
            uint32_t w1, w2;
            SYM_TRACE(4, s, 0);
            wait_for(s, R_E | R_Y2 | R_S, &w1, &w2, kNapShort);
            SYM_TRACE(4, s, 1);
            P3_LAP(p3_wait);
            const uint32_t f2 = flags_of_last(w2, s);
            if (f2 & Y2F_LEAVE) stop_at = s;
            if ((f2 & (Y2F_END | Y2F_LOCK)) && s >= 1u) {
                const uint32_t from_y2 = fb2box[((s - 1u) & 1u) * LY::fb_words + lane];
                const bool superseded = (last_msg & (YM_DROP | YM_ADJUSTED)) != 0u;
#ifdef SYM_Y1_SELECT
                Q.L.flags |= ((from_y2 & FB_SQLOCK) && !superseded) ? (uint32_t)F_SQ_LOCK : 0u;
                const bool y2_end = (from_y2 & FB_END) && !superseded;
                if (__builtin_expect(__builtin_amdgcn_ballot_w64(y2_end) != 0ull, 0)) Q.end_masked(y2_end);
#else
                if ((from_y2 & FB_SQLOCK) && !superseded) Q.L.flags |= F_SQ_LOCK;
                if ((from_y2 & FB_END) && !superseded) Q.end();
#endif
            }
            last_msg = 0u;
            uint32_t flags = 0u;
            if (s >= 2u && s <= last_y1_step) {
                const lds_u32 *sb = symbox + ((s - 1u) & 1u) * LY::sym_words + lane;
                const uint32_t hdr = sb[0], zero_w = sb[kWave], sym_w = sb[2 * kWave];
                uint32_t msg = 0u, fbv = 0u;
#ifdef SYM_Y1_SELECT
                {
                    const bool valid = (hdr & 1u) && !PROF_SKIP(P, 16);
                    const uint32_t off = hdr >> 8;
                    const float zero = __uint_as_float(zero_w), sym = __uint_as_float(sym_w);
                    if (P.trace_cap && valid) {
                        const State S = fresh_state();
                        const uint64_t counter = counter0 + (int64_t)row_l + (uint64_t)sym_index(s - 1u, off) + 1u;
                        const uint32_t n = S.trace_n[c];
                        if (n < P.trace_cap) {
                            float *t = S.trace + ((size_t)c * P.trace_cap + n) * 4;
                            t[0] = zero; t[1] = sym; t[2] = __uint_as_float(sb[3 * kWave]); t[3] = __uint_as_float(sb[4 * kWave]);
                            S.trace_idx[(size_t)c * P.trace_cap + n] = counter;
                        }
                        S.trace_n[c] = n + 1;
                    }
                    msg = Q.symbol_masked(P, valid, zero, sym, off, &fbv);
                }
#else
                if ((hdr & 1u) && !PROF_SKIP(P, 16)) {
                    const uint32_t off = hdr >> 8;
                    const float zero = __uint_as_float(zero_w), sym = __uint_as_float(sym_w);
                    if (P.trace_cap) {
                        const State S = fresh_state();
                        const uint64_t counter = counter0 + (int64_t)row_l + (uint64_t)sym_index(s - 1u, off) + 1u;
                        const uint32_t n = S.trace_n[c];
                        if (n < P.trace_cap) {
                            float *t = S.trace + ((size_t)c * P.trace_cap + n) * 4;
                            t[0] = zero; t[1] = sym; t[2] = __uint_as_float(sb[3 * kWave]); t[3] = __uint_as_float(sb[4 * kWave]);
                            S.trace_idx[(size_t)c * P.trace_cap + n] = counter;
                        }
                        S.trace_n[c] = n + 1;
                    }
                    msg = Q.symbol(P, zero, sym, off, &fbv);
                }
#endif
                ybox[(s & 1u) * kWave + lane] = msg;
                last_msg = msg;
                if (__builtin_amdgcn_ballot_w64(fbv != 0u) != 0ull) {
                    uint32_t u1, u2;
                    wait_for(s, R_S, &u1, &u2, kNapLong);
                    fb1box[(s & 1u) * LY::fb_words + lane] = fbv; flags = Y1F_ANY;
                }
            }
            if (s + 1u == n_steps) flagbox[lane] = Q.L.flags & (F_AGC_LOCKED | F_BW_LOCKED | F_SQ_LOCK | F_EQ_MODE_MASK | F_EQ_BITS_MASK);
            SYM_TRACE(4, s, 2);
            peek();
            publish(s, flags, flags_before);
            flags_before = flags;
            P3_LAP(p3_work);
            if (s == stop_at) { left = true; break; }
        }
        SYM_REPORT(4);
        if (left || gave_up()) return;
        const State S = fresh_state();
        S.sq_data[c] = Q.L.sq_data; S.sq_power[c] = Q.L.sq_power; S.sq_phist[c] = Q.L.sq_phist;
        S.sq_fill[c] = Q.L.sq_fill; S.sq_clock[c] = Q.L.sq_clock; S.sq_symbols[c] = symbols0 + (uint64_t)(Q.nsym - (uint32_t)symbols0);
        S.eq_word[c] = Q.L.eq_word; S.eq_count[c] = Q.L.eq_count;
        if (hist_copy) {
#pragma unroll 4
            for (int i = 0; i < kSquelchHist; ++i) S.sq_hist[(size_t)i * C + c] = *Q.hptr((uint32_t)i);
        }
#pragma unroll
        for (int i = 0; i < NFF; ++i) {
            S.eq_ffc[i * C + c] = Q.ffc[i]; S.eq_ffw[i * C + c] = Q.ffw[i];
            S.eq_snap_ffc[i * C + c] = Q.sffc[i]; S.eq_snap_ffw[i * C + c] = Q.sffw[i];
        }
#pragma unroll
        for (int i = 0; i < NFB; ++i) {
            S.eq_fbc[i * C + c] = Q.fbc[i]; S.eq_fbw[i * C + c] = Q.fbw[i];
            S.eq_snap_fbc[i * C + c] = Q.sfbc[i]; S.eq_snap_fbw[i * C + c] = Q.sfbw[i];
        }
    } else {
        sym_setprio<sym_prio<NT>(6)>(P);
        Lane L;
        SymFramer F;
        uint8_t *fr_rows;
        { const State S0 = fresh_state(); lane_load(L, S0, c); fr_rows = S0.fr_msg; }
        F.st = fr_state(L); F.last = (L.flags & F_LINK_MASK) >> F_LINK_SHIFT;
        F.word = L.fr_word; F.count = L.fr_count; F.invalid = L.fr_invalid; F.len = L.fr_len;
        uint8_t *const row = fr_rows + (size_t)c * kBurstCap;
        Output O{};
        { const Output Of = fresh_output(); O.n_events = Of.n_events; O.bursts = Of.bursts; O.burst_cap = Of.burst_cap; }
        lds_barrier();
        P3_T0();
        uint32_t stop_at = 0xffffffffu, flags_before = 0u;
        bool left = false, lane_done = false, leave_posted = false;
        for (uint32_t s = 0; s < n_steps; ++s) {
            uint32_t w1, w2;
            SYM_TRACE(5, s, 0);
            wait_for(s, R_Y1 | R_S | R_T | R_A | R_E, &w1, &w2, kNapShort);
            SYM_TRACE(5, s, 1);
            P3_LAP(p3_wait);
            uint32_t flags = 0u;
            if (s >= 3u && s <= last_y2_step) {
                const uint32_t m = PROF_SKIP(P, 1024) ? 0u : ybox[((s - 1u) & 1u) * kWave + lane];
                uint32_t fbv = 0, burst_len = 0, io1 = 0xffffffffu;
                bool emit = false;
                const uint32_t link = sym_framer_step(P, F, row, m, &burst_len, &fbv, &emit);
                const bool want_slot = emit & (link == 3u);
                const uint32_t io0 = (m & YM_VALID) ? (1u | (link << 1) | (emit ? 8u : 0u) | (((m >> YM_OFF_SHIFT) & kSymOffMask) << 4)) : 0u;
                uint64_t pend = __builtin_amdgcn_ballot_w64(want_slot);
                lds_u32 *io = iobox + (s & 1u) * LY::io_words + lane;
                if (pend != 0ull) {
                    const uint32_t n_new = (uint32_t)__popcll(pend);
                    uint32_t base = 0;
                    if (lane == 0u) base = atomicAdd(O.n_events + 1, n_new);
                    base = (uint32_t)__builtin_amdgcn_readfirstlane((int)base);
                    uint32_t k = 0;
                    while (pend != 0ull) {
                        const int j = __builtin_ctzll(pend);
                        pend &= pend - 1ull;
                        const uint32_t b = base + k++;
                        const uint32_t cj = (uint32_t)__builtin_amdgcn_readlane((int)c, j);
                        if (b < O.burst_cap) {
                            const uint32_t *src = reinterpret_cast<const uint32_t *>(fr_rows + (size_t)cj * kBurstCap);
                            uint32_t *dst = reinterpret_cast<uint32_t *>(O.bursts + (size_t)b * kBurstCap);
                            constexpr uint32_t kWords = (uint32_t)kBurstCap / 4u, kPer = (kWords + kWave - 1u) / kWave;
                            uint32_t t[kPer];
#pragma unroll
                            for (uint32_t i = 0; i < kPer; ++i) { const uint32_t w = lane + i * kWave; t[i] = w < kWords ? src[w] : 0u; }
#pragma unroll
                            for (uint32_t i = 0; i < kPer; ++i) { const uint32_t w = lane + i * kWave; if (w < kWords) dst[w] = t[i]; }
                            if ((int)lane == j) io1 = b;
                        } else {
                            if (lane == 0u) atomicOr(O.n_events + 2, 2u);
                            if ((int)lane == j) io1 = 0xffffffffu;
                        }
                    }
                    io[kWave] = io1; io[2 * kWave] = burst_len;
                }
                io[0] = io0;
                const bool any_end = __builtin_amdgcn_ballot_w64((fbv & FB_VALID) != 0u) != 0ull;
                const bool any_lock = __builtin_amdgcn_ballot_w64((fbv & FB_SQLOCK) != 0u) != 0ull;
                if (any_end || any_lock) fb2box[(s & 1u) * LY::fb_words + lane] = fbv;
                flags = (any_end ? Y2F_END : 0u) | (any_lock ? Y2F_LOCK : 0u);
                if (may_leave && !leave_posted) {
                    const uint32_t blk = min(s - 3u, n_blocks - 1u);
                    if (!lane_done && blk + 1u >= n_nominal && F.last == 0u && (xl == nullptr || blk < avail_l)) {
                        lane_done = true;
                        K.handover[c] = counter0 + (int64_t)row_l + (uint64_t)(blk + 1u) * kB;
                        donebox[lane] = 1u;
                    }
                    if (__builtin_amdgcn_ballot_w64(!lane_done) == 0ull) { flags |= Y2F_LEAVE; leave_posted = true; stop_at = s + 1u; }
                }
            }
            SYM_TRACE(5, s, 2);
            peek();
            publish(s, flags, flags_before);
            flags_before = flags;
            P3_LAP(p3_work);
            if (s == stop_at) { left = true; break; }
        }
        SYM_REPORT(5);
        SYM_COUNT(18, 1);
        SYM_COUNT(19, left ? stop_at + 1u : n_steps);
        if (left || gave_up()) return;
        uint32_t w1, w2;
        wait_for(n_steps, R_A | R_E | R_Y1, &w1, &w2, kNapShort);
        if (gave_up()) return;
        const uint32_t flags_out = (F.st << F_FR_STATE_SHIFT) | (F.last << F_LINK_SHIFT) | (phasebox[lane] & F_TED_PHASE) | (againbox[lane] & F_TICK_AGAIN) | flagbox[lane];
        const State S1 = fresh_state();
        S1.fr_word[c] = F.word; S1.fr_count[c] = F.count; S1.fr_invalid[c] = F.invalid;
        S1.fr_len[c] = F.len; S1.flags[c] = flags_out;
    }
}

#if !defined(SAME_PROFILE) && !defined(SAME_SYM_TL)
#define SYM_SPLIT_TU 1
#endif
static_assert(SymLayout<42>::B == kSymStep22 && SymLayout<92>::B == kSymStepHi && SymLayout<84>::B == kSymStepHi && SymLayout<42>::NBLK == kSymRingSteps &&
              SymLayout<92>::NBLK == kSymRingSteps, "same_select.h decides with these steps and this ring");

template <int NT, int NFF, int NFB, typename SampleT>
static hipError_t launch_sym_one(const Params &P, const State &S, const Output &O, const float4 *taps, const SampleT *x,
                                 uint32_t n_blocks, uint64_t counter0, hipStream_t stream, const PipeChunks &K)
{
    constexpr uint32_t kSymHalves = (uint32_t)SymLayout<NT>::HALVES;
    constexpr size_t lds = (size_t)kSymHalves * SymLayout<NT>::lds_bytes;
    static_assert(lds <= 160u * 1024u, "one workgroup per CU");
    const bool cm = K.n_chunks > 1u && K.col_row0 != nullptr;
    if (cm && (!std::is_same<SampleT, float>::value || NT != 42)) return hipErrorInvalidValue;
    if (K.n_chunks > 1u && (K.in_channels % kWave) != 0u) return hipErrorInvalidValue;
    if (n_blocks == 0u) return hipSuccess;
    auto go = [&](auto kernel) -> hipError_t {
        if (lds > 64u * 1024u) {
            static std::mutex mu;
            static std::set<std::pair<const void *, int>> opted_in;
            int dev = 0;
            if (hipGetDevice(&dev) != hipSuccess) return hipErrorInvalidDevice;
            const std::pair<const void *, int> key(reinterpret_cast<const void *>(kernel), dev);
            std::lock_guard<std::mutex> lock(mu);
            if (opted_in.find(key) == opted_in.end()) {
                const hipError_t e = hipFuncSetAttribute(key.first, hipFuncAttributeMaxDynamicSharedMemorySize, (int)lds);
                if (e != hipSuccess) return e;
                opted_in.insert(key);
            }
        }
        hipLaunchKernelGGL(kernel, dim3((P.n_channels / kWave + kSymHalves - 1u) / kSymHalves), dim3(kSymHalves * kSymRoles * kWave), lds, stream, P, S, O, taps, x, n_blocks, counter0, K);
        return hipGetLastError();
    };
    if constexpr (std::is_same<SampleT, float>::value && NT == 42) {
        if (cm) return go(demod_sym_kernel<NT, NFF, NFB, float, 1>);
    }
    return go(demod_sym_kernel<NT, NFF, NFB, SampleT, 0>);
}

template <typename SampleT>
static hipError_t launch_sym_hi_t(const Params &P, const State &S, const Output &O, const float4 *taps, const SampleT *x,
                                  uint32_t n_blocks, uint64_t counter0, hipStream_t stream, const PipeChunks &K)
{
    const bool eq = P.eq_nff == 6u && P.eq_nfb == 4u;
    if (standard_rate_taps(P) == 92u)
        return eq ? launch_sym_one<92, 6, 4, SampleT>(P, S, O, taps, x, n_blocks, counter0, stream, K) : launch_sym_one<92, 1, 1, SampleT>(P, S, O, taps, x, n_blocks, counter0, stream, K);
    return eq ? launch_sym_one<84, 6, 4, SampleT>(P, S, O, taps, x, n_blocks, counter0, stream, K) : launch_sym_one<84, 1, 1, SampleT>(P, S, O, taps, x, n_blocks, counter0, stream, K);
}
#if defined(SYM_TU_HI)
#if defined(SYM_SPLIT_TU)
hipError_t launch_demod_sym_hi(const Params &P, const State &S, const Output &O, const float4 *taps, const float *x,
                               uint32_t n_blocks, uint64_t counter0, hipStream_t stream, const PipeChunks &K)
{ return launch_sym_hi_t<float>(P, S, O, taps, x, n_blocks, counter0, stream, K); }
hipError_t launch_demod_sym_hi(const Params &P, const State &S, const Output &O, const float4 *taps, const int16_t *x,
                               uint32_t n_blocks, uint64_t counter0, hipStream_t stream, const PipeChunks &K)
{ return launch_sym_hi_t<int16_t>(P, S, O, taps, x, n_blocks, counter0, stream, K); }
#endif
#else
#if defined(SYM_SPLIT_TU)
hipError_t launch_demod_sym_hi(const Params &P, const State &S, const Output &O, const float4 *taps, const float *x,
                               uint32_t n_blocks, uint64_t counter0, hipStream_t stream, const PipeChunks &K);
hipError_t launch_demod_sym_hi(const Params &P, const State &S, const Output &O, const float4 *taps, const int16_t *x,
                               uint32_t n_blocks, uint64_t counter0, hipStream_t stream, const PipeChunks &K);
#else
template <typename SampleT>
static hipError_t launch_demod_sym_hi(const Params &P, const State &S, const Output &O, const float4 *taps, const SampleT *x,
                                      uint32_t n_blocks, uint64_t counter0, hipStream_t stream, const PipeChunks &K)
{ return launch_sym_hi_t<SampleT>(P, S, O, taps, x, n_blocks, counter0, stream, K); }
#endif
template <typename SampleT>
static hipError_t launch_sym_t(const Params &P, const State &S, const Output &O, const float4 *taps, const SampleT *x,
                               uint32_t n_blocks, uint64_t counter0, hipStream_t stream, const PipeChunks &K)
{
    if (!sym_kernel_supported(P)) return hipErrorInvalidValue;
    const bool eq = P.eq_nff == 6u && P.eq_nfb == 4u;
    if (standard_rate_taps(P) == 42u)
        return eq ? launch_sym_one<42, 6, 4, SampleT>(P, S, O, taps, x, n_blocks, counter0, stream, K) : launch_sym_one<42, 1, 1, SampleT>(P, S, O, taps, x, n_blocks, counter0, stream, K);
    return launch_demod_sym_hi(P, S, O, taps, x, n_blocks, counter0, stream, K);
}
// ... 14 lines not shown
```

### sameold_amd/csrc/same_launch.h

```cpp
#pragma once

#include <hip/hip_runtime.h>

#include "same_capture_dev.h"
#include "same_device.h"
#include "same_select.h"

namespace same {

hipError_t launch_demod(const Params &P, const State &S, const Output &O, const float4 *taps,
                        const float *x, uint32_t n_samples, uint64_t counter0, hipStream_t stream);
hipError_t launch_demod(const Params &P, const State &S, const Output &O, const float4 *taps,
                        const int16_t *x, uint32_t n_samples, uint64_t counter0, hipStream_t stream);
hipError_t launch_demod_ragged(const Params &P, const State &S, const Output &O, const float4 *taps, const float *x,
                               uint32_t n_rows, const uint32_t *counts, uint32_t row_sub, uint64_t counter0, hipStream_t stream);
hipError_t launch_demod_ragged(const Params &P, const State &S, const Output &O, const float4 *taps, const int16_t *x,
                               uint32_t n_rows, const uint32_t *counts, uint32_t row_sub, uint64_t counter0, hipStream_t stream);
hipError_t launch_demod_pipe(const Params &P, const State &S, const Output &O, const float4 *taps,
                             const float *x, uint32_t n_blocks, uint64_t counter0, hipStream_t stream,
                             const PipeChunks &chunks = PipeChunks{}, bool relaxed = false);
hipError_t launch_demod_pipe(const Params &P, const State &S, const Output &O, const float4 *taps,
                             const int16_t *x, uint32_t n_blocks, uint64_t counter0, hipStream_t stream,
                             const PipeChunks &chunks = PipeChunks{}, bool relaxed = false);
hipError_t launch_demod_sym(const Params &P, const State &S, const Output &O, const float4 *taps,
                            const float *x, uint32_t n_blocks, uint64_t counter0, hipStream_t stream,
                            const PipeChunks &chunks = PipeChunks{});
hipError_t launch_demod_sym(const Params &P, const State &S, const Output &O, const float4 *taps,
                            const int16_t *x, uint32_t n_blocks, uint64_t counter0, hipStream_t stream,
                            const PipeChunks &chunks = PipeChunks{});
hipError_t launch_demod_relaxed(const Params &P, const State &S, const Output &O, const float4 *taps,
                                const float *x, uint32_t n_blocks, uint64_t counter0, hipStream_t stream,
                                const PipeChunks &chunks = PipeChunks{});
hipError_t launch_demod_relaxed(const Params &P, const State &S, const Output &O, const float4 *taps,
                                const int16_t *x, uint32_t n_blocks, uint64_t counter0, hipStream_t stream,
                                const PipeChunks &chunks = PipeChunks{});
hipError_t launch_demod_fast(const Params &P, const State &S, const Output &O, const float4 *taps,
                             const float *x, uint32_t n_blocks, uint64_t counter0, hipStream_t stream);
hipError_t launch_demod_fast(const Params &P, const State &S, const Output &O, const float4 *taps,
                             const int16_t *x, uint32_t n_blocks, uint64_t counter0, hipStream_t stream);
hipError_t launch_counters(uint32_t *dev, uint32_t *host_mapped, int publish, hipStream_t stream);
hipError_t launch_event_sort(const DevEvent *ev, const uint32_t *counters, uint32_t cap, uint32_t n_bins, uint32_t *cnt, uint32_t *first,
                             DevEvent *sorted, hipStream_t stream, bool cnt_is_zero = false);
hipError_t launch_init_state(const Params &P, const State &S, int is_reset, hipStream_t stream, uint32_t first_col = 0);
hipError_t launch_reset_columns(const Params &P, const State &S, const uint32_t *cols, uint32_t n, hipStream_t stream);
hipError_t launch_copy_state_columns(const StateArrayDesc *desc, uint32_t n_desc, uint32_t src_channels,
                                     uint32_t dst_channels, const uint32_t *src_col, uint32_t n_cols, hipStream_t stream,
                                     uint32_t src_base = 0);
hipError_t launch_chunk_final_column(const uint64_t *handover, uint32_t in_channels, ChunkGeom g, uint32_t *final_col,
                                     hipStream_t stream);
hipError_t launch_chunk_final_column_pc(const uint64_t *handover, const uint32_t *own_start, uint32_t in_channels, uint32_t n_chunks,
                                        uint64_t counter0, uint32_t *final_col, hipStream_t stream);
hipError_t launch_fill_u64(uint64_t *p, size_t n, uint64_t v, hipStream_t stream);
hipError_t launch_cast_i16_f32(const int16_t *in, float *out, size_t n, hipStream_t stream);
hipError_t launch_tp_prologue(void *blob, const void *fresh, size_t bytes, uint64_t *handover, uint32_t *sort_cnt, uint32_t n_cols,
                              uint32_t *counters, hipStream_t stream);
struct TpPlan {
    uint32_t channels, n_chunks, block_len, warmup_samples, whole_samples;
    uint64_t in_samples;
    uint32_t scout_blocks;
};
hipError_t launch_tp_plan(const float *x, const TpPlan &g, float *energy, uint32_t *own_start, uint32_t *row0,
                          uint32_t *nominal, uint32_t *perm, uint32_t *wg_blocks, bool sorted, hipStream_t stream,
                          uint32_t *perm_out = nullptr, uint32_t *wg_blocks_out = nullptr, bool pairs = false);
hipError_t launch_transpose(const float *in, float *out, uint32_t n_channels, uint32_t n_samples,
                            hipStream_t stream);
hipError_t launch_transpose(const int16_t *in, int16_t *out, uint32_t n_channels, uint32_t n_samples,
                            hipStream_t stream);

constexpr uint32_t kMessageLogOverflow = 8u;
struct TransportLaunch {
    uint32_t n_channels, input_rate;
    const uint32_t *first;
    DevEvent *sorted;
    const uint32_t *counters;
    const uint8_t *bursts; uint32_t burst_cap;
    void *hot, *cold;
    uint64_t *wake_sample;
    DevMessage *near; uint32_t near_cap;
    DevMessage *log; uint32_t log_cap;
    uint32_t *log_cursor, *overflow;
    cap::Launch cap;
};
size_t transport_hot_bytes();
size_t transport_cold_bytes();
hipError_t launch_transport(const TransportLaunch &T, hipStream_t stream);
hipError_t launch_transport_ragged(const TransportLaunch &T, const uint32_t *counts, uint32_t row_sub, uint32_t n_rows, hipStream_t stream);
hipError_t launch_transport_reset(void *hot, void *cold, uint32_t n_channels, const uint32_t *cols, uint32_t n, int fresh,
                                  hipStream_t stream, void *capture_rec = nullptr);
hipError_t launch_capture(const cap::Span *spans, cap::Cursors *cur, uint32_t span_cap, float *pool, uint64_t pool_cap,
                          const float *x, uint32_t n_channels, uint32_t n_rows, cap::Cursors *host, hipStream_t stream);
hipError_t launch_capture(const cap::Span *spans, cap::Cursors *cur, uint32_t span_cap, float *pool, uint64_t pool_cap,
                          const int16_t *x, uint32_t n_channels, uint32_t n_rows, cap::Cursors *host, hipStream_t stream);

struct SynthParams {
    uint32_t n_channels;
    uint32_t input_rate;
    uint64_t seed;
    float noise_sigma;
    uint32_t flags;
};
hipError_t launch_synth(const SynthParams &sp, float *x, size_t n_samples, hipStream_t stream);
struct TrialParams {
    uint32_t n_trials;
    uint32_t first_trial;
    uint32_t input_rate;
    uint32_t n_grid;
    uint64_t seed;
    float ebn0_db_lo, ebn0_db_step;
};
hipError_t launch_trials(const TrialParams &tp, float *x, size_t n_samples, hipStream_t stream);
uint32_t synth_payload(uint64_t seed, uint32_t channel, uint8_t *out, uint32_t cap);

}
```

### sameold_amd/csrc/same_tp_plan.cpp

```cpp
#include "same_tp_plan.h"

#include <algorithm>

namespace same {

TpCut tp_uniform_cut(const Params &P, const Mode &m, const Request &rq, const TpConfig &cfg, size_t n, uint64_t counter0,
                     uint32_t column_cap, bool channel_major)
{
    TpCut cut;
    const uint32_t C = P.n_channels;
    const double sps = (double)P.input_rate / 520.83;
    auto fill = [&](uint32_t K, uint32_t fb) -> bool {
        const uint32_t warm = cfg.warmup ? cfg.warmup : (uint32_t)(64.0 * sps + 0.5);
        const uint32_t WB = (warm + fb - 1u) / fb;
        const uint64_t TB = n / fb;
        if (TB <= WB) return false;
        const uint64_t SB = (TB - WB) / K;
        const uint64_t min_own = cfg.min_own ? cfg.min_own : 4ull * WB * fb;
        if (SB == 0 || SB * fb < min_own) return false;
        cut.geom.counter0 = counter0;
        cut.geom.n_chunks = K; cut.geom.block_len = fb; cut.geom.stride_blocks = (uint32_t)SB; cut.geom.warmup_blocks = WB;
        cut.pc.n_chunks = K; cut.pc.in_channels = C; cut.pc.stride_blocks = (uint32_t)SB; cut.pc.nominal_blocks = (uint32_t)SB + WB;
        return true;
    };
    const TpRule rule = tp_rule(P, m, rq, cfg.max_chunks, column_cap, channel_major);
    for (uint32_t K = rule.k_max; K >= 2u; --K) {
        Choice c;
        if (tp_candidate(P, rule, K, c) && fill(K, c.block_len)) { cut.n_chunks = K; cut.choice = c; return cut; }
    }
    return cut;
}

TpCut tp_native_cut(const Params &P, const Mode &m, const Request &rq, const TpConfig &cfg, size_t n_call, uint64_t counter0)
{
    if (n_call > kMaxLaunchSamples || P.ntaps != 42u) return TpCut{};
    return tp_uniform_cut(P, m, rq, cfg, n_call, counter0, tp_native_column_cap(P, m, cfg.max_chunks), true);
}

TpNative tp_native_plan(const Params &P, const TpConfig &cfg, const TpCut &cut, size_t n_call, uintptr_t base)
{
    TpNative np;
    if (cut.n_chunks < 2u) return np;
    const uint32_t C = P.n_channels, columns = cut.n_chunks * C, fb = cut.geom.block_len;
    const Family family = cut.choice.family;
    const bool wave = family == Family::kWaveRelaxed;
    const Params Pv = wide_params(P, columns, is_fastmath(family), true);
    const size_t n = n_call - n_call % fb;
    if (n_call % 4 != 0 || (base & 15u) != 0u || n < 64u * (size_t)kScoutBlock || n / kScoutBlock > 7000u || cut.n_chunks > 63u || C % kWave != 0u) return np;
    if (wave ? fb % 2 != 0 : (fb % 4 != 0 || pipe_workgroup_channels(Pv) != (uint32_t)kWave)) return np;
    np.qualifies = true;
    const double sps = (double)P.input_rate / 520.83;
    const uint32_t warm = cfg.warmup ? cfg.warmup : (uint32_t)(40.0 * sps + 0.5);
    np.warmup_samples = std::min(cut.geom.warmup_blocks, (warm + fb - 1u) / fb) * fb;
    np.whole_samples = (uint32_t)n; np.in_samples = n_call;
    np.scout_blocks = (uint32_t)(n / kScoutBlock);
    np.energy_floats = (size_t)C * np.scout_blocks;
    np.pair_groups = cfg.sort_mode == 2 && family == Family::kSym;
    np.sort_mode = np.pair_groups ? 0 : (cfg.sort_mode >= 0 ? (cfg.sort_mode ? 1 : 0) : (tp_more_than_one_round(columns) ? 1 : 0));
    np.lpt = np.sort_mode != 0 || np.pair_groups;
    np.need_hist = np.lpt && family == Family::kSym;
    np.hist_floats = np.need_hist ? (size_t)columns * kSquelchHist : 0;
    const size_t groups = columns / kWave;
    TpGeomWords &w = np.words;
    w.own_start = 0; w.row0 = columns; w.nominal = 2 * (size_t)columns; w.perm = 3 * (size_t)columns; w.wg = 4 * (size_t)columns;
    w.wg2 = w.wg + groups; w.perm2 = w.wg2 + 2 * groups;
    w.total = w.perm2 + columns;
    w.harvest = 2 * (size_t)columns;
    return np;
}

OutputCaps output_caps(const Params &P, size_t n_samples, size_t n_columns, bool dev_transport, bool audio, size_t near_cap, size_t msg_cap)
{
    OutputCaps o;
    const size_t n_ch = n_columns ? n_columns : P.n_channels;
    const double symbols = (double)n_samples * 520.83 / (double)P.input_rate;
    const size_t per_chan_events = (size_t)(symbols / 8.0) + 16;
    const size_t per_chan_bursts = (size_t)(symbols / 160.0) + 4;
    o.events = std::min<size_t>(per_chan_events * n_ch, 0x7fffffffu / sizeof(DevEvent));
    o.bursts = std::min<size_t>(per_chan_bursts * n_ch, 0x7fffffffu / kBurstCap);
    if (dev_transport && !n_columns) {
        o.messages = std::min<size_t>(o.bursts + 2 * n_ch, 0x7fffffffu / sizeof(DevMessage));
        o.near = near_cap ? near_cap : std::max<uint32_t>(4096u, (uint32_t)(n_ch / 4u));
        if (audio) o.spans = std::min<size_t>(n_ch + o.near + std::max(msg_cap, o.messages), 0x7fffffffu / kSpanBytes);
    }
    o.bins = n_ch;
    o.sort_words = 2 * n_ch + 1 + event_sort_extra_words((uint32_t)n_ch);
    return o;
}

}
```

### sameold_amd/csrc/same_tp_plan.h

```cpp
#pragma once

#include <stddef.h>
#include <stdint.h>

#include "same_config.h"
#include "same_device.h"
#include "same_select.h"

namespace same {

#ifndef SAME_SCOUT_BLOCK
#define SAME_SCOUT_BLOCK 256
#endif
constexpr uint32_t kScoutBlock = SAME_SCOUT_BLOCK;
constexpr uint32_t kScanThreads = 1024;
inline uint32_t event_sort_extra_words(uint32_t n_bins) { return (n_bins + kScanThreads - 1u) / kScanThreads; }

constexpr size_t kMaxLaunchSamples = (size_t)1 << 22;
inline size_t max_launch_samples(uint32_t input_rate) { return kMaxLaunchSamples < (size_t)input_rate * 45 ? kMaxLaunchSamples : (size_t)input_rate * 45; }

struct TpConfig {
    uint32_t max_chunks = 0, min_own = 0, warmup = 0;
    int sort_mode = -1;
    int knob_plan_stream = 0;
    int knob_prologue = 0;
};

struct TpCut {
    uint32_t n_chunks = 1;
    Choice choice;
    ChunkGeom geom{};
    PipeChunks pc{};
};
TpCut tp_uniform_cut(const Params &P, const Mode &m, const Request &rq, const TpConfig &cfg, size_t n, uint64_t counter0,
                     uint32_t column_cap = kTpColumnCap, bool channel_major = false);

TpCut tp_native_cut(const Params &P, const Mode &m, const Request &rq, const TpConfig &cfg, size_t n_call, uint64_t counter0);
struct TpGeomWords {
    size_t own_start = 0, row0 = 0, nominal = 0, perm = 0, wg = 0, wg2 = 0, perm2 = 0;
    size_t total = 0;
    size_t harvest = 0;
};
struct TpNative {
    bool qualifies = false;
    uint32_t whole_samples = 0;
    uint32_t warmup_samples = 0, scout_blocks = 0;
    uint64_t in_samples = 0;
    int sort_mode = 0;
    bool pair_groups = false;
    bool lpt = false;
    bool need_hist = false;
    size_t hist_floats = 0, energy_floats = 0;
    TpGeomWords words;
};
TpNative tp_native_plan(const Params &P, const TpConfig &cfg, const TpCut &cut, size_t n_call, uintptr_t base);
inline bool tp_plan_beside(const TpConfig &cfg, bool own_stream) { return own_stream && cfg.knob_plan_stream >= 0; }

constexpr size_t kSpanBytes = 32;
struct OutputCaps {
    size_t events = 0, bursts = 0;
    size_t messages = 0, near = 0, spans = 0;
    size_t bins = 0, sort_words = 0;
};
OutputCaps output_caps(const Params &P, size_t n_samples, size_t n_columns, bool dev_transport, bool audio, size_t near_cap, size_t msg_cap);
inline size_t tp_output_samples(size_t n, const PipeChunks &pc, uint32_t block_len)
{
    const size_t m = 3 * (size_t)pc.nominal_blocks * block_len + 65536;
    return n < m ? n : m;
}

}
```

### sameold_amd/receiver.py

```python
from __future__ import annotations

import ctypes as C
import os
import sys
from typing import Iterator, List, Optional, Sequence

import numpy as np

_HERE = os.path.dirname(os.path.abspath(__file__))
LIB_PATH = os.path.join(_HERE, f"libsame_rx.{os.environ['SAME_LIB_VARIANT']}.so" if os.environ.get("SAME_LIB_VARIANT") else "libsame_rx.so")

LINK_NO_CARRIER, LINK_SEARCHING, LINK_READING, LINK_BURST = 0, 1, 2, 3
TRANSPORT_IDLE, TRANSPORT_ASSEMBLING, TRANSPORT_MSG_START, TRANSPORT_MSG_END, TRANSPORT_MSG_ERR = 16, 17, 18, 19, 20
LAYOUT_TIME_MAJOR, LAYOUT_CHANNEL_MAJOR = 0, 1
BATCH_LINK_ONLY, BATCH_TRACE_SYMBOLS, BATCH_GENERIC_KERNEL, BATCH_TIME_PARALLEL, BATCH_RELAXED, BATCH_CALL_INVARIANT = 1, 2, 4, 8, 16, 32
BATCH_MESSAGES_ONLY = 64
TP_EVENT_TOLERANCE_SYMBOLS = 2
STREAM_OWN = (1 << 64) - 1
EVENT_MAX_BYTES = 288
AUDIO_FIRST, AUDIO_END_MESSAGE, AUDIO_END_FLUSH, AUDIO_END_RESET, AUDIO_TRUNCATED = 1, 2, 4, 8, 16
AUDIO_END = AUDIO_END_MESSAGE | AUDIO_END_FLUSH | AUDIO_END_RESET

ERRORS = {-1: "EINVAL", -2: "EDCLEN", -3: "EAGCLIMITS", -4: "EEQORDER", -5: "ENODEVICE",
          -6: "EHIP", -7: "EOVERFLOW", -8: "ENOMEM", -9: "ERATE", -10: "EKERNEL"}
# ... 66 lines not shown


def _share_hip_runtime_with_torch() -> None:
    import importlib.util
    if "torch" in sys.modules:
        return
    try:
        spec = importlib.util.find_spec("torch")
    except (ImportError, ValueError):
        spec = None
    if spec is None or not spec.origin:
        return
    cand = os.path.join(os.path.dirname(spec.origin), "lib", "libamdhip64.so")
    if os.path.exists(cand):
        try:
            C.CDLL(cand, mode=C.RTLD_GLOBAL)
        except OSError:
            pass


def load_library() -> C.CDLL:
    global _lib
    if _lib is not None:
        return _lib
    if not os.path.exists(LIB_PATH):
        raise SameError(-5, f"{LIB_PATH} is missing: run `python -m sameold_amd.build` "
                            "(hipcc, gfx950); there is no CPU implementation to fall back to")
    _share_hip_runtime_with_torch()
    L = C.CDLL(LIB_PATH)
    P, vp, u32, u64, f32 = C.POINTER, C.c_void_p, C.c_uint32, C.c_uint64, C.c_float

    def sig(name, res, *args):
        fn = getattr(L, name)
        fn.restype = res
        fn.argtypes = list(args)

    sig("same_last_error", C.c_char_p)
    sig("same_rx_abi_version", u32)
    sig("same_rx_builder_new", vp, u32)
    sig("same_rx_builder_default", vp)
    sig("same_rx_builder_clone", vp, vp)
    sig("same_rx_builder_free", None, vp)
    sig("same_rx_builder_with_dc_blocker_length", None, vp, f32)
    sig("same_rx_builder_with_agc_bandwidth", None, vp, f32)
    sig("same_rx_builder_with_agc_gain_limits", None, vp, f32, f32)
    sig("same_rx_builder_with_timing_bandwidth", None, vp, f32, f32)
    sig("same_rx_builder_with_timing_max_deviation", None, vp, f32)
    sig("same_rx_builder_with_squelch_power", None, vp, f32, f32)
    sig("same_rx_builder_with_squelch_bandwidth", None, vp, f32)
    sig("same_rx_builder_with_preamble_max_errors", None, vp, u32)
    sig("same_rx_builder_with_adaptive_equalizer", None, vp, u32, u32, f32, f32)
    sig("same_rx_builder_without_adaptive_equalizer", None, vp)
    sig("same_rx_builder_with_frame_prefix_max_errors", None, vp, u32)
    sig("same_rx_builder_with_frame_max_invalid", None, vp, u32)
    sig("same_rx_builder_input_rate", u32, vp)
    sig("same_rx_builder_dc_blocker_length", f32, vp)
    sig("same_rx_builder_agc_bandwidth", f32, vp)
    sig("same_rx_builder_agc_gain_limits", None, vp, P(f32))
    sig("same_rx_builder_timing_bandwidth", None, vp, P(f32), P(f32))
    sig("same_rx_builder_timing_max_deviation", f32, vp)
    sig("same_rx_builder_squelch_power", None, vp, P(f32), P(f32))
    sig("same_rx_builder_squelch_bandwidth", f32, vp)
    sig("same_rx_builder_preamble_max_errors", u32, vp)
    sig("same_rx_builder_adaptive_equalizer", C.c_int, vp, P(u32), P(u32), P(f32), P(f32))
    sig("same_rx_builder_frame_prefix_max_errors", u32, vp)
    sig("same_rx_builder_frame_max_invalid", u32, vp)

    sig("same_batch_new", C.c_int, vp, u32, C.c_int, u32, P(vp))
    sig("same_batch_free", None, vp)
    sig("same_batch_reset", C.c_int, vp)
    sig("same_batch_reset_channels", C.c_int, vp, P(u32), C.c_size_t)
    sig("same_batch_channel_input_sample_counter", u64, vp, u32)
    sig("same_batch_input_rate", u32, vp)
    sig("same_batch_n_channels", u32, vp)
    sig("same_batch_input_sample_counter", u64, vp)
    sig("same_batch_device", C.c_int, vp)
    sig("same_batch_process_device", C.c_int, vp, vp, C.c_size_t, u32, vp)
    sig("same_batch_order_after", C.c_int, vp, vp)
    sig("same_batch_set_call_window", C.c_int, vp, C.c_uint32)
    sig("same_batch_time_parallel_config", C.c_int, vp, u32, u32, u32)
    sig("same_batch_time_parallel_chunks", u32, vp)
    sig("same_batch_time_parallel_per_channel", C.c_int, vp)
    sig("same_batch_debug_tp_plan", C.c_int, vp, P(TpPlanInfo), vp, C.c_size_t, vp, C.c_size_t, vp, C.c_size_t, vp, C.c_size_t)
    sig("same_batch_transport_on_device", C.c_int, vp)
    sig("same_batch_set_audio_capture", C.c_int, vp, C.c_size_t)
    sig("same_batch_peek_audio", C.c_int, vp, P(P(AudioChunk)), P(C.c_size_t))
    sig("same_batch_drop_audio", C.c_int, vp, C.c_size_t)
    sig("same_rx_source_hash", C.c_char_p)
    sig("same_batch_process_device_i16", C.c_int, vp, vp, C.c_size_t, u32, vp)
    sig("same_batch_process_host", C.c_int, vp, vp, C.c_size_t, u32)
    sig("same_batch_process_host_i16", C.c_int, vp, vp, C.c_size_t, u32)
    sig("same_batch_process_device_ragged", C.c_int, vp, vp, C.c_size_t, P(u32), u32, vp)
    sig("same_batch_process_device_ragged_i16", C.c_int, vp, vp, C.c_size_t, P(u32), u32, vp)
    sig("same_batch_process_host_ragged", C.c_int, vp, vp, C.c_size_t, P(u32), u32)
    sig("same_batch_process_host_ragged_i16", C.c_int, vp, vp, C.c_size_t, P(u32), u32)
    sig("same_batch_flush", C.c_int, vp)
    sig("same_batch_sync", C.c_int, vp)
    sig("same_batch_poll_events", C.c_int, vp, P(Event), C.c_size_t, P(C.c_size_t), P(C.c_size_t))
    sig("same_batch_pending_events", C.c_size_t, vp)
    sig("same_batch_peek_events", C.c_int, vp, P(P(Event)), P(C.c_size_t))
    sig("same_batch_drop_events", C.c_int, vp, C.c_size_t)
    sig("same_batch_pack_bursts", C.c_int, vp, u32, vp, C.c_size_t, P(C.c_size_t))
    sig("same_batch_read_trace", C.c_int, vp, u32, P(SymbolTrace), C.c_size_t, P(C.c_size_t))
    sig("same_batch_last_kernel_ms", C.c_int, vp, P(f32))
    sig("same_batch_last_demod_kernel_ms", C.c_int, vp, P(f32))
    sig("same_batch_set_kernel_timing", None, vp, C.c_int)
    sig("same_batch_kernel_name", C.c_char_p, vp)

    sig("same_rx_build", C.c_int, vp, C.c_int, P(vp))
    sig("same_rx_free", None, vp)
    sig("same_rx_process", C.c_int, vp, vp, C.c_size_t, P(C.c_size_t), P(Event))
    sig("same_rx_flush", C.c_int, vp, P(Event))
    sig("same_rx_reset", C.c_int, vp)
    sig("same_rx_input_rate", u32, vp)
    sig("same_rx_input_sample_counter", u64, vp)

    sig("same_synth_afsk_device", C.c_int, vp, u32, C.c_size_t, u32, u64, f32, u32, C.c_int, vp)
    sig("same_synth_payload", u32, u64, u32, C.c_char_p, u32)
    _lib = L
    return L


def _check(rc: int):
    if rc < 0:
        raise SameError(rc, load_library().same_last_error().decode(errors="replace"))
    return rc


class SameReceiverBuilder:

    def __init__(self, input_rate: int = 22050):
        self._L = load_library()
        self._h = C.c_void_p(self._L.same_rx_builder_new(input_rate))

    def __del__(self):
        if getattr(self, "_h", None):
            self._L.same_rx_builder_free(self._h)
            self._h = None

    def with_dc_blocker_length(self, length: float):
        self._L.same_rx_builder_with_dc_blocker_length(self._h, length); return self

    def with_agc_bandwidth(self, bw: float):
        self._L.same_rx_builder_with_agc_bandwidth(self._h, bw); return self

    def with_agc_gain_limits(self, mn: float, mx: float):
        self._L.same_rx_builder_with_agc_gain_limits(self._h, mn, mx); return self

    def with_timing_bandwidth(self, unlocked: float, locked: float):
        self._L.same_rx_builder_with_timing_bandwidth(self._h, unlocked, locked); return self

    def with_timing_max_deviation(self, max_dev: float):
        self._L.same_rx_builder_with_timing_max_deviation(self._h, max_dev); return self

    def with_squelch_power(self, open_: float, close: float):
        self._L.same_rx_builder_with_squelch_power(self._h, open_, close); return self

    def with_squelch_bandwidth(self, bw: float):
        self._L.same_rx_builder_with_squelch_bandwidth(self._h, bw); return self

    def with_preamble_max_errors(self, n: int):
        self._L.same_rx_builder_with_preamble_max_errors(self._h, n); return self

    def with_adaptive_equalizer(self, nfeedforward=6, nfeedback=4, relaxation=0.05, regularization=1.0e-6):
        self._L.same_rx_builder_with_adaptive_equalizer(self._h, nfeedforward, nfeedback, relaxation, regularization)
        return self
# ... 66 lines not shown
                                 messages_only)


class SameBatchReceiver:

    def __init__(self, builder: SameReceiverBuilder, n_channels: int, device: int = 0,
                 link_only: bool = False, trace_symbols: bool = False, generic_kernel: bool = False,
                 time_parallel: bool = False, relaxed: bool = False, call_invariant: bool = False, messages_only: bool = False):
        self._L = load_library()
        h = C.c_void_p()
        flags = ((BATCH_LINK_ONLY if link_only else 0) | (BATCH_TRACE_SYMBOLS if trace_symbols else 0)
                 | (BATCH_GENERIC_KERNEL if generic_kernel else 0) | (BATCH_TIME_PARALLEL if time_parallel else 0)
                 | (BATCH_RELAXED if relaxed else 0) | (BATCH_CALL_INVARIANT if call_invariant else 0)
                 | (BATCH_MESSAGES_ONLY if messages_only else 0))
        _check(self._L.same_batch_new(builder._h, n_channels, device, flags, C.byref(h)))
        self._h = h
        self._inflight = []

    def __del__(self):
        if getattr(self, "_h", None):
            self._L.same_batch_free(self._h)
            self._h = None

    @property
    def n_channels(self) -> int:
        return self._L.same_batch_n_channels(self._h)

    def input_rate(self) -> int:
        return self._L.same_batch_input_rate(self._h)

    def input_sample_counter(self) -> int:
        return self._L.same_batch_input_sample_counter(self._h)

    def kernel_name(self) -> str:
        return self._L.same_batch_kernel_name(self._h).decode()

    def set_call_window(self, samples: int) -> None:
        _check(self._L.same_batch_set_call_window(self._h, int(samples)))

    def reset(self):
        _check(self._L.same_batch_reset(self._h))

    def reset_channels(self, channels) -> None:
        if hasattr(channels, "detach"):
            channels = channels.detach().numpy()
        arr = np.atleast_1d(np.asarray(channels))
        if arr.size and (arr.dtype.kind not in "iu" or arr.min() < 0 or arr.max() >= 1 << 32):
            raise ValueError("channels must be non-negative integers")
        arr = np.ascontiguousarray(arr.reshape(-1), dtype=np.uint32)
        _check(self._L.same_batch_reset_channels(self._h, arr.ctypes.data_as(C.POINTER(C.c_uint32)), arr.size))

    def channel_input_sample_counter(self, channel: int) -> int:
        if not 0 <= channel < self.n_channels:
            raise IndexError(f"channel {channel} of {self.n_channels}")
        return int(self._L.same_batch_channel_input_sample_counter(self._h, channel))

    def time_parallel_config(self, max_chunks: int = 0, min_own_samples: int = 0, warmup_samples: int = 0):
        _check(self._L.same_batch_time_parallel_config(self._h, max_chunks, min_own_samples, warmup_samples))

    def time_parallel_chunks(self) -> int:
        return self._L.same_batch_time_parallel_chunks(self._h)

    def transport_on_device(self) -> int:
        return int(self._L.same_batch_transport_on_device(self._h))

    def time_parallel_per_channel(self) -> bool:
        return bool(self._L.same_batch_time_parallel_per_channel(self._h))

    def debug_tp_plan(self) -> dict:
        info = TpPlanInfo()
        none = C.c_void_p()
        _check(self._L.same_batch_debug_tp_plan(self._h, C.byref(info), none, 0, none, 0, none, 0, none, 0))
        columns = info.n_chunks * info.channels
        energy = np.empty((info.channels, info.scout_blocks), np.float32)
        geom = np.empty(info.w_total, np.uint32)
        handover = np.empty((info.n_chunks, info.channels), np.uint64)
        final_col = np.empty(info.channels, np.uint32)
        _check(self._L.same_batch_debug_tp_plan(self._h, C.byref(info), C.c_void_p(energy.ctypes.data), energy.size,
                                                C.c_void_p(geom.ctypes.data), geom.size, C.c_void_p(handover.ctypes.data), columns,
                                                C.c_void_p(final_col.ctypes.data), final_col.size))
        out = {name: int(getattr(info, name)) for name, _ in TpPlanInfo._fields_ if name != "reserved"}
        out.update(energy=energy, geom=geom, handover=handover, final_col=final_col)
        return out

    def set_audio_capture(self, samples_per_launch: int) -> None:
        _check(self._L.same_batch_set_audio_capture(self._h, int(samples_per_launch)))

    def poll_audio(self) -> list:
        ptr, n = C.POINTER(AudioChunk)(), C.c_size_t()
        _check(self._L.same_batch_peek_audio(self._h, C.byref(ptr), C.byref(n)))
        out = []
        for i in range(n.value):
            ch = ptr[i]
            k = int(ch.n_samples)
            a = np.ctypeslib.as_array(ch.samples, shape=(k,)).copy() if k else np.zeros(0, np.float32)
            out.append((int(ch.channel), int(ch.sample_counter), int(ch.flags), a))
        if n.value:
            _check(self._L.same_batch_drop_audio(self._h, n.value))
        return out

    def process_device_ptr(self, ptr: int, n_samples: int, layout: int = LAYOUT_TIME_MAJOR,
                           stream: Optional[int] = None, i16: bool = False):
        fn = self._L.same_batch_process_device_i16 if i16 else self._L.same_batch_process_device
        _check(fn(self._h, C.c_void_p(ptr), n_samples, layout, C.c_void_p(STREAM_OWN if stream is None else stream)))

    def order_after(self, producer_stream: int):
        _check(self._L.same_batch_order_after(self._h, C.c_void_p(producer_stream)))

    def process_tensor(self, x, layout: int = LAYOUT_TIME_MAJOR, stream: Optional[int] = None):
        import torch
        assert x.is_cuda and x.is_contiguous()
        if layout == LAYOUT_TIME_MAJOR:
            n, ch = x.shape
        else:
            ch, n = x.shape
        assert ch == self.n_channels
        if x.dtype not in (torch.float32, torch.int16):
            raise TypeError("float32 or int16 input")
        if stream is None:
            self.order_after(torch.cuda.current_stream(x.device).cuda_stream)
        self._inflight.append(x)
        self.process_device_ptr(x.data_ptr(), n, layout, stream, x.dtype == torch.int16)
        if len(self._inflight) > 2:
            del self._inflight[0]

    def process_host(self, x: np.ndarray, layout: int = LAYOUT_TIME_MAJOR):
        x = np.ascontiguousarray(x)
        if x.ndim == 1:
            x = x.reshape(-1, 1) if layout == LAYOUT_TIME_MAJOR else x.reshape(1, -1)
        n, ch = x.shape if layout == LAYOUT_TIME_MAJOR else x.shape[::-1]
        assert ch == self.n_channels, (ch, self.n_channels)
        if x.dtype == np.int16:
            _check(self._L.same_batch_process_host_i16(self._h, C.c_void_p(x.ctypes.data), n, layout))
        else:
            x = np.ascontiguousarray(x, dtype=np.float32)
            _check(self._L.same_batch_process_host(self._h, C.c_void_p(x.ctypes.data), n, layout))

    def _ragged_counts(self, counts):
        if hasattr(counts, "detach"):
            counts = counts.detach().cpu().numpy()
        a = np.asarray(counts)
        if a.ndim != 1 or a.shape[0] != self.n_channels:
            raise SameError(-1, f"ragged call: {a.shape} counts for {self.n_channels} channels; nothing was consumed")
        if a.size and (a.min() < 0 or a.max() > 0xffffffff):
            raise SameError(-1, "ragged call: a count is out of range; nothing was consumed")
        return np.ascontiguousarray(a, dtype=np.uint32)

    def process_ragged(self, x, counts, layout: int = LAYOUT_TIME_MAJOR, stream: Optional[int] = None):
        import torch
        assert x.is_cuda and x.is_contiguous()
        if layout == LAYOUT_TIME_MAJOR:
            n, ch = x.shape
        else:
            ch, n = x.shape
        assert ch == self.n_channels
        if x.dtype not in (torch.float32, torch.int16):
            raise TypeError("float32 or int16 input")
        k = self._ragged_counts(counts)
        if stream is None:
            self.order_after(torch.cuda.current_stream(x.device).cuda_stream)
        self._inflight.append(x)
        fn = self._L.same_batch_process_device_ragged_i16 if x.dtype == torch.int16 else self._L.same_batch_process_device_ragged
        try:
            _check(fn(self._h, C.c_void_p(x.data_ptr()), n, k.ctypes.data_as(C.POINTER(C.c_uint32)), layout,
                      C.c_void_p(STREAM_OWN if stream is None else stream)))
        except SameError:
# ... 243 lines not shown
```

Before: 468,600.

## Store time-parallel sym state at scheduled position via inverse permutation map

When columns are permuted for LPT/pair scheduling in the sym kernel, per-lane state is now indexed by scheduled position instead of original column. An inverse position map is built after planning and applied in the state copy-in/copy-out kernels, which replaces the gathered per-column accesses and the squelch history scratch copy-in/out. It also adds a sort_mode 3 that regroups pairs with sorting when one round suffices. The trade is an extra small map kernel plus indirection in the state copies, in exchange for coalesced state accesses in the main kernel.

```diff
diff --git a/include/same_rx.h b/include/same_rx.h
--- a/include/same_rx.h
+++ b/include/same_rx.h
@@ -160,6 +160,7 @@
 } same_tp_plan_info;
 int same_batch_debug_tp_plan(same_batch *rx, same_tp_plan_info *info, float *energy, size_t energy_cap, uint32_t *geom,
                              size_t geom_cap, uint64_t *handover, size_t handover_cap, uint32_t *final_col, size_t final_col_cap);
+int same_batch_debug_tp_position_map(same_batch *rx, uint32_t *columns, uint32_t *inv, size_t inv_cap);
 
 int same_batch_transport_on_device(const same_batch *rx);
 
diff --git a/sameold_amd/csrc/same_batch.cpp b/sameold_amd/csrc/same_batch.cpp
--- a/sameold_amd/csrc/same_batch.cpp
+++ b/sameold_amd/csrc/same_batch.cpp
@@ -80,6 +80,8 @@
         same::TpPlan plan{};
         uint64_t plan_counter0 = 0;
         bool plan_sorted = false, plan_lpt = false, plan_pairs = false;
+        same::DevBuf<uint32_t> d_pos_map;
+        bool pos_mapped = false;
         same::CoherentBuf<uint32_t> h_reset;
         same::CoherentBuf<uint32_t> h_counts;
         same::PinnedBuf<uint64_t> h_wake_up;
@@ -112,7 +114,6 @@
         uint32_t n_desc = 0;
         same::DevBuf<uint32_t> d_final_col;
         same::DevBuf<float> d_energy;
-        same::DevBuf<float> d_hist;
         same::Event ev_plan_prev; bool plan_recorded = false;
         uint32_t last_chunks = 1;
         bool last_per_channel = false;
@@ -576,7 +577,8 @@
     return SAME_OK;
 }
 
-int tp_start(same_batch *rx, same_batch::Slot &sl, uint32_t columns, const char *layout, hipStream_t stream, bool *sort_bins_empty)
+int tp_start(same_batch *rx, same_batch::Slot &sl, uint32_t columns, const char *layout, hipStream_t stream, bool *sort_bins_empty,
+             const uint32_t *pos_map)
 {
     same_batch::TimePar &tp = rx->tp;
     const uint32_t C = rx->P.n_channels;
@@ -586,12 +588,12 @@
         *sort_bins_empty = sl.sort_bins == columns;
     } else {
         HIP_TRY(same::launch_counters(sl.d_counters, sl.h_counters.dev(), 0, stream));
-        HIP_TRY(same::launch_init_state(tp.Pv, tp.Sv, 0, stream, C));
+        HIP_TRY(same::launch_init_state(tp.Pv, tp.Sv, 0, stream, pos_map ? 0u : C));
         HIP_TRY(same::launch_fill_u64(sl.d_handover, columns, same::kNoHandover, stream));
     }
     if (rx->debug) std::fprintf(stderr, "[same] time-parallel launch: %u columns (%s), start-up: %s\n", columns, layout,
                                 tp.cfg.knob_prologue >= 0 ? "prologue kernel" : "separate launches");
-    HIP_TRY(same::launch_copy_state_columns(tp.d_desc_in, tp.n_desc, C, columns, nullptr, C, stream));
+    HIP_TRY(same::launch_copy_state_columns(tp.d_desc_in, tp.n_desc, C, columns, nullptr, C, stream, 0, pos_map, nullptr));
     return SAME_OK;
 }
 
@@ -631,6 +633,8 @@
     if (tp.plan_recorded) HIP_TRY(hipStreamWaitEvent(ps, tp.ev_plan_prev, 0));
     HIP_TRY(same::launch_tp_plan(d_x, plan, tp.d_energy, g + w.own_start, g + w.row0, g + w.nominal, g + w.perm, g + w.wg, np.sort_mode != 0, ps,
                                  np.lpt ? g + w.perm2 : nullptr, np.lpt ? g + w.wg2 : nullptr, np.pair_groups));
+    sl.pos_mapped = np.pos_map;
+    if (np.pos_map) HIP_TRY(same::launch_tp_position_map(g + w.perm2, sl.d_pos_map, plan.n_chunks * plan.channels, ps));
     HIP_TRY(tp.ev_plan_prev.ensure());
     HIP_TRY(hipEventRecord(tp.ev_plan_prev, ps));
     tp.plan_recorded = true;
@@ -641,7 +645,6 @@
     pc.col_row0 = g + w.row0; pc.col_nominal = g + w.nominal;
     pc.wg_blocks = g + (np.lpt ? w.wg2 : w.wg); pc.col_perm = np.lpt ? g + w.perm2 : nullptr;
     pc.in_samples = np.in_samples; pc.whole_samples = np.whole_samples;
-    pc.hist_scratch = np.need_hist ? tp.d_hist.get() : nullptr;
     return SAME_OK;
 }
 
@@ -667,7 +670,7 @@
         HIP_TRY(sl.d_geom.ensure(np->words.total));
         HIP_TRY(sl.h_geom.ensure(np->words.harvest));
         HIP_TRY(tp.d_energy.ensure(np->energy_floats));
-        if (np->need_hist) HIP_TRY(tp.d_hist.ensure(np->hist_floats));
+        if (np->pos_map) HIP_TRY(sl.d_pos_map.ensure(columns));
         sl.words = np->words;
     }
     rc = begin_timing(rx, sl, stream);
@@ -675,7 +678,9 @@
     const float *xf = nullptr;
     if constexpr (std::is_same_v<SampleT, float>) xf = x;
     if (np && (rc = tp_plan_boundaries(rx, sl, cut, *np, xf, stream, pc)) != SAME_OK) return rc;
-    rc = tp_start(rx, sl, columns, np ? "channel-major" : "time-major", stream, sort_bins_empty);
+    const uint32_t *pos_map = np && np->pos_map ? sl.d_pos_map.get() : nullptr;
+    if (!np) sl.pos_mapped = false;
+    rc = tp_start(rx, sl, columns, np ? "channel-major" : "time-major", stream, sort_bins_empty, pos_map);
     if (rc) return rc;
     sl.have_k = np && sl.timed;
     if (sl.have_k) HIP_TRY(hipEventRecord(sl.ev_k0, stream));
@@ -685,7 +690,7 @@
     if (sl.have_k) HIP_TRY(hipEventRecord(sl.ev_k1, stream));
     if (np) HIP_TRY(same::launch_chunk_final_column_pc(sl.d_handover, sl.d_geom + np->words.own_start, C, geom.n_chunks, rx->counter, tp.d_final_col, stream));
     else HIP_TRY(same::launch_chunk_final_column(sl.d_handover, C, geom, tp.d_final_col, stream));
-    HIP_TRY(same::launch_copy_state_columns(tp.d_desc_out, tp.n_desc, columns, C, tp.d_final_col, C, stream));
+    HIP_TRY(same::launch_copy_state_columns(tp.d_desc_out, tp.n_desc, columns, C, tp.d_final_col, C, stream, 0, nullptr, pos_map));
     if (n_whole < n_call) {
         rc = np ? demod_tail_corner(rx, O, xf + n_whole, n_call, n_call - n_whole, rx->counter + n_whole, stream)
                 : demod_tail(rx, O, x + n_whole * C, n_call - n_whole, rx->counter + n_whole, stream);
@@ -1501,6 +1506,23 @@
     return SAME_OK;
 }
 
+int same_batch_debug_tp_position_map(same_batch *rx, uint32_t *columns, uint32_t *inv, size_t inv_cap)
+{
+    if (!rx || !columns) return fail(SAME_EINVAL, "null argument");
+    if (rx->launch_seq == 0) return fail(SAME_EINVAL, "no launch yet");
+    const same_batch::Slot &sl = rx->slot[(rx->launch_seq - 1) & 1];
+    if (!sl.chunked || !sl.per_channel) return fail(SAME_EINVAL, "the last launch had no per-channel plan");
+    if (rx->slot[0].in_flight || rx->slot[1].in_flight) return fail(SAME_EINVAL, "a launch is in flight: same_batch_sync first");
+    const size_t n = sl.pos_mapped ? (size_t)sl.plan.n_chunks * sl.plan.channels : 0;
+    *columns = (uint32_t)n;
+    if (!n || !inv) return SAME_OK;
+    if (inv_cap < n) return fail(SAME_EINVAL, "a read-back buffer is too small");
+    if (n > sl.d_pos_map.size()) return fail(SAME_EINVAL, "the plan's buffers are gone");
+    HIP_TRY(hipSetDevice(rx->device));
+    HIP_TRY(hipMemcpy(inv, sl.d_pos_map, n * sizeof(uint32_t), hipMemcpyDeviceToHost));
+    return SAME_OK;
+}
+
 const char *same_batch_kernel_name(const same_batch *rx)
 {
     return rx ? same::family_name(rx->last_family, rx->P.block_len) : "";
diff --git a/sameold_amd/csrc/same_device.h b/sameold_amd/csrc/same_device.h
--- a/sameold_amd/csrc/same_device.h
+++ b/sameold_amd/csrc/same_device.h
@@ -105,7 +105,6 @@
     const uint32_t *col_nominal;
     const uint32_t *wg_blocks;
     const uint32_t *col_perm;
-    float *hist_scratch;
     uint64_t in_samples;
     uint32_t whole_samples;
 };
diff --git a/sameold_amd/csrc/same_kernels.hip b/sameold_amd/csrc/same_kernels.hip
--- a/sameold_amd/csrc/same_kernels.hip
+++ b/sameold_amd/csrc/same_kernels.hip
@@ -451,12 +451,16 @@
 }
 
 __global__ void copy_state_columns_kernel(const StateArrayDesc *desc, uint32_t Csrc, uint32_t Cdst,
-                                          const uint32_t *src_col, uint32_t n_cols, uint32_t src_base)
-{
-    const uint32_t col = blockIdx.x * blockDim.x + threadIdx.x;
-    if (col >= n_cols) return;
+                                          const uint32_t *src_col, uint32_t n_cols, uint32_t src_base,
+                                          const uint32_t *__restrict__ dst_map, const uint32_t *__restrict__ src_map)
+{
+    const uint32_t col0 = blockIdx.x * blockDim.x + threadIdx.x;
+    if (col0 >= n_cols) return;
     const StateArrayDesc d = desc[blockIdx.y];
-    const uint32_t sc = src_col ? src_col[col] : col + src_base;
+    uint32_t sc = src_col ? src_col[col0] : col0 + src_base;
+    if (src_map) sc = src_map[sc];
+    const uint32_t col = dst_map ? dst_map[col0] : col0;
+    if (col >= Cdst || sc >= Csrc) return;
     const uint32_t w = d.elem_words;
     const uint32_t *src = reinterpret_cast<const uint32_t *>(d.src);
     uint32_t *dst = reinterpret_cast<uint32_t *>(d.dst);
@@ -468,10 +472,10 @@
 }
 hipError_t launch_copy_state_columns(const StateArrayDesc *desc, uint32_t n_desc, uint32_t src_channels,
                                      uint32_t dst_channels, const uint32_t *src_col, uint32_t n_cols, hipStream_t stream,
-                                     uint32_t src_base)
+                                     uint32_t src_base, const uint32_t *dst_map, const uint32_t *src_map)
 {
     hipLaunchKernelGGL(copy_state_columns_kernel, dim3((n_cols + 255) / 256, n_desc, 16), dim3(256), 0, stream, desc,
-                       src_channels, dst_channels, src_col, n_cols, src_base);
+                       src_channels, dst_channels, src_col, n_cols, src_base, dst_map, src_map);
     return hipGetLastError();
 }
 __global__ void chunk_final_column_kernel(const uint64_t *handover, uint32_t C, ChunkGeom g, uint32_t *final_col)
@@ -690,6 +694,18 @@
     perm_out[pos * kWave + lane] = perm[w * kWave + lane];
     if (lane == 0) wg_blocks_out[pos] = wg_blocks[w];
 }
+__global__ void tp_position_map_kernel(const uint32_t *__restrict__ perm, uint32_t *__restrict__ inv, uint32_t n)
+{
+    const uint32_t p = blockIdx.x * blockDim.x + threadIdx.x;
+    if (p >= n) return;
+    const uint32_t v = perm[p];
+    if (v < n) inv[v] = p;
+}
+hipError_t launch_tp_position_map(const uint32_t *perm, uint32_t *inv, uint32_t columns, hipStream_t stream)
+{
+    hipLaunchKernelGGL(tp_position_map_kernel, dim3((columns + 255) / 256), dim3(256), 0, stream, perm, inv, columns);
+    return hipGetLastError();
+}
 hipError_t launch_tp_plan(const float *x, const TpPlan &g, float *energy, uint32_t *own_start, uint32_t *row0,
                           uint32_t *nominal, uint32_t *perm, uint32_t *wg_blocks, bool sorted, hipStream_t stream,
                           uint32_t *perm_out, uint32_t *wg_blocks_out, bool pairs)
diff --git a/sameold_amd/csrc/same_kernels_sym.hip b/sameold_amd/csrc/same_kernels_sym.hip
--- a/sameold_amd/csrc/same_kernels_sym.hip
+++ b/sameold_amd/csrc/same_kernels_sym.hip
@@ -928,7 +928,8 @@
     const uint32_t vwg = blockIdx.x * kSymHalves + half;
     if (vwg * kWave >= C) return;
     float *lds = lds_all + half * (uint32_t)(LY::lds_bytes / sizeof(float));
-    const uint32_t c = (K.n_chunks > 1u && K.col_perm) ? K.col_perm[vwg * kWave + lane] : vwg * kWave + lane;
+    const uint32_t pos = vwg * kWave + lane;
+    const uint32_t c = (K.n_chunks > 1u && K.col_perm) ? K.col_perm[pos] : pos;
     uint32_t cin = c, Cin = C, n_nominal = n_blocks;
     bool may_leave = false;
     int32_t row_l = 0;
@@ -1030,7 +1031,7 @@
     if (role == 0u) {
         sym_setprio<sym_prio<NT>(0)>(P);
         SymAgc<NT> M;
-        { const State S = fresh_state(); M.load(P, S, c, C, counter0, wcol); }
+        { const State S = fresh_state(); M.load(P, S, pos, C, counter0, wcol); }
         lds_barrier();
         P3_T0();
         uint32_t stop_at = 0xffffffffu;
@@ -1068,14 +1069,14 @@
         }
         SYM_REPORT(0);
         if (left || gave_up()) return;
-        { const State S = fresh_state(); M.store(P, S, c, C, counter1, wcol); }
+        { const State S = fresh_state(); M.store(P, S, pos, C, counter1, wcol); }
     } else if (role == 1u) {
         sym_setprio<sym_prio<NT>(1)>(P);
         if constexpr (NT != 42) {
             static_assert(CMODE == 0 && kNSUB == 2, "time-major rows, two sub-blocks a step");
             SymDcRot<SampleT, NT> D;
             const uint32_t n_sub = n_blocks * (uint32_t)kNSUB;
-            { const State S = fresh_state(); D.load(S, x, c, C, cin, Cin, counter0, n_sub); }
+            { const State S = fresh_state(); D.load(S, x, pos, C, cin, Cin, counter0, n_sub); }
             donebox[lane] = 0u;
             D.template sub<0>(P, wcol, x, 0u, n_sub, cin, Cin);
             D.template sub<1>(P, wcol, x, 1u, n_sub, cin, Cin);
@@ -1111,14 +1112,14 @@
             }
             SYM_REPORT(1);
             if (left || gave_up()) return;
-            { const State S = fresh_state(); D.store(S, c, C, counter1, n_sub - 1u); }
+            { const State S = fresh_state(); D.store(S, pos, C, counter1, n_sub - 1u); }
             return;
         } else {
         using Dc = SymDc<SampleT, CMODE, NT>;
         Dc D;
         D.xl = xl; D.avail = avail_l;
         const uint32_t n_sub = n_blocks * (uint32_t)kNSUB;
-        { const State S = fresh_state(); D.load(S, x, c, C, cin, Cin, counter0, n_sub); }
+        { const State S = fresh_state(); D.load(S, x, pos, C, cin, Cin, counter0, n_sub); }
         donebox[lane] = 0u;
         auto sub_tm = [&](uint32_t q, auto pb_) __attribute__((always_inline)) {
             typename Dc::Pairs X;
@@ -1178,7 +1179,7 @@
         }
         SYM_REPORT(1);
         if (left || gave_up()) return;
-        { const State S = fresh_state(); D.store(S, c, C, counter1); }
+        { const State S = fresh_state(); D.store(S, pos, C, counter1); }
         }
     } else if (role == 2u) {
         sym_setprio<sym_prio<NT>(2)>(P);
@@ -1193,8 +1194,8 @@
         X.tk = tkbox + lane;
         {
             const State S = fresh_state();
-            lane_load(L, S, c);
-            X.ring_load(P, S, c);
+            lane_load(L, S, pos);
+            X.ring_load(P, S, pos);
         }
         const State Snone{};
         Output O{};
@@ -1262,8 +1263,8 @@
         if (left || gave_up()) return;
         {
             const State S = fresh_state();
-            S.tk_next[c] = L.tk_next; S.tk_last[c] = L.tk_last; S.wake_fired[c] = L.wake_fired;
-            X.ring_store(P, S, c);
+            S.tk_next[pos] = L.tk_next; S.tk_last[pos] = L.tk_last; S.wake_fired[pos] = L.wake_fired;
+            X.ring_store(P, S, pos);
         }
     } else if (role == 3u) {
         sym_setprio<sym_prio<NT>(4)>(P);
@@ -1271,7 +1272,7 @@
         std::conditional_t<NT == 42, SymTaps<42>, SymHalfTaps<NT, NT / 4, NT / 2>> TP;
         TP.load(taps);
         Lane L;
-        { const State S = fresh_state(); lane_load(L, S, c); }
+        { const State S = fresh_state(); lane_load(L, S, pos); }
         const float inv_spt = 1.0f / P.samples_per_ted;
         int cstar = next_fire_count(L.until_next_ted, L.ted_clock);
         int rel = cstar - (int)L.ted_clock - 1;
@@ -1419,36 +1420,31 @@
         L.ted_clock = (uint32_t)((int)cstar_f - rel - 1);
         {
             const State S = fresh_state();
-            S.until_next_ted[c] = L.until_next_ted; S.ted_clock[c] = L.ted_clock;
-            S.ted_h0[c] = L.h0; S.ted_h1[c] = L.h1; S.ted_h2[c] = L.h2;
-            S.period_avg[c] = L.period_avg; S.period_inst[c] = L.period_inst;
+            S.until_next_ted[pos] = L.until_next_ted; S.ted_clock[pos] = L.ted_clock;
+            S.ted_h0[pos] = L.h0; S.ted_h1[pos] = L.h1; S.ted_h2[pos] = L.h2;
+            S.period_avg[pos] = L.period_avg; S.period_inst[pos] = L.period_inst;
         }
     } else if (role == 4u) {
         sym_setprio<sym_prio<NT>(5)>(P);
         SymSquelch<NFF, NFB> Q;
         uint64_t symbols0;
-        const bool hist_copy = K.n_chunks > 1u && K.col_perm != nullptr && K.hist_scratch != nullptr;
         {
             const State S = fresh_state();
-            lane_load(Q.L, S, c);
+            lane_load(Q.L, S, pos);
             symbols0 = Q.L.sq_symbols;
             Q.nsym = (uint32_t)symbols0;
-            Q.hbase = reinterpret_cast<char *>(hist_copy ? K.hist_scratch : S.sq_hist);
-            Q.hcol4 = (hist_copy ? vwg * kWave + lane : c) * 4u;
+            Q.hbase = reinterpret_cast<char *>(S.sq_hist);
+            Q.hcol4 = pos * 4u;
             Q.hrow4 = C * 4u;
-            if (hist_copy) {
-#pragma unroll 4
-                for (int i = 0; i < kSquelchHist; ++i) *Q.hptr((uint32_t)i) = S.sq_hist[(size_t)i * C + c];
-            }
 #pragma unroll
             for (int i = 0; i < NFF; ++i) {
-                Q.ffc[i] = S.eq_ffc[i * C + c]; Q.ffw[i] = S.eq_ffw[i * C + c];
-                Q.sffc[i] = S.eq_snap_ffc[i * C + c]; Q.sffw[i] = S.eq_snap_ffw[i * C + c];
+                Q.ffc[i] = S.eq_ffc[i * C + pos]; Q.ffw[i] = S.eq_ffw[i * C + pos];
+                Q.sffc[i] = S.eq_snap_ffc[i * C + pos]; Q.sffw[i] = S.eq_snap_ffw[i * C + pos];
             }
 #pragma unroll
             for (int i = 0; i < NFB; ++i) {
-                Q.fbc[i] = S.eq_fbc[i * C + c]; Q.fbw[i] = S.eq_fbw[i * C + c];
-                Q.sfbc[i] = S.eq_snap_fbc[i * C + c]; Q.sfbw[i] = S.eq_snap_fbw[i * C + c];
+                Q.fbc[i] = S.eq_fbc[i * C + pos]; Q.fbw[i] = S.eq_fbw[i * C + pos];
+                Q.sfbc[i] = S.eq_snap_fbc[i * C + pos]; Q.sfbw[i] = S.eq_snap_fbw[i * C + pos];
             }
             const uint32_t pslot = (2u * Q.nsym) & 63u;
             Q.nxt0 = *Q.hptr((pslot + 16u) & 63u); Q.nxt1 = *Q.hptr((pslot + 17u) & 63u);
@@ -1491,13 +1487,13 @@
                     if (P.trace_cap && valid) {
                         const State S = fresh_state();
                         const uint64_t counter = counter0 + (int64_t)row_l + (uint64_t)sym_index(s - 1u, off) + 1u;
-                        const uint32_t n = S.trace_n[c];
+                        const uint32_t n = S.trace_n[pos];
                         if (n < P.trace_cap) {
-                            float *t = S.trace + ((size_t)c * P.trace_cap + n) * 4;
+                            float *t = S.trace + ((size_t)pos * P.trace_cap + n) * 4;
                             t[0] = zero; t[1] = sym; t[2] = __uint_as_float(sb[3 * kWave]); t[3] = __uint_as_float(sb[4 * kWave]);
-                            S.trace_idx[(size_t)c * P.trace_cap + n] = counter;
+                            S.trace_idx[(size_t)pos * P.trace_cap + n] = counter;
                         }
-                        S.trace_n[c] = n + 1;
+                        S.trace_n[pos] = n + 1;
                     }
                     msg = Q.symbol_masked(P, valid, zero, sym, off, &fbv);
                 }
@@ -1508,13 +1504,13 @@
                     if (P.trace_cap) {
                         const State S = fresh_state();
                         const uint64_t counter = counter0 + (int64_t)row_l + (uint64_t)sym_index(s - 1u, off) + 1u;
-                        const uint32_t n = S.trace_n[c];
+                        const uint32_t n = S.trace_n[pos];
                         if (n < P.trace_cap) {
-                            float *t = S.trace + ((size_t)c * P.trace_cap + n) * 4;
+                            float *t = S.trace + ((size_t)pos * P.trace_cap + n) * 4;
                             t[0] = zero; t[1] = sym; t[2] = __uint_as_float(sb[3 * kWave]); t[3] = __uint_as_float(sb[4 * kWave]);
-                            S.trace_idx[(size_t)c * P.trace_cap + n] = counter;
+                            S.trace_idx[(size_t)pos * P.trace_cap + n] = counter;
                         }
-                        S.trace_n[c] = n + 1;
+                        S.trace_n[pos] = n + 1;
                     }
                     msg = Q.symbol(P, zero, sym, off, &fbv);
                 }
@@ -1538,32 +1534,28 @@
         SYM_REPORT(4);
         if (left || gave_up()) return;
         const State S = fresh_state();
-        S.sq_data[c] = Q.L.sq_data; S.sq_power[c] = Q.L.sq_power; S.sq_phist[c] = Q.L.sq_phist;
-        S.sq_fill[c] = Q.L.sq_fill; S.sq_clock[c] = Q.L.sq_clock; S.sq_symbols[c] = symbols0 + (uint64_t)(Q.nsym - (uint32_t)symbols0);
-        S.eq_word[c] = Q.L.eq_word; S.eq_count[c] = Q.L.eq_count;
-        if (hist_copy) {
-#pragma unroll 4
-            for (int i = 0; i < kSquelchHist; ++i) S.sq_hist[(size_t)i * C + c] = *Q.hptr((uint32_t)i);
-        }
+        S.sq_data[pos] = Q.L.sq_data; S.sq_power[pos] = Q.L.sq_power; S.sq_phist[pos] = Q.L.sq_phist;
+        S.sq_fill[pos] = Q.L.sq_fill; S.sq_clock[pos] = Q.L.sq_clock; S.sq_symbols[pos] = symbols0 + (uint64_t)(Q.nsym - (uint32_t)symbols0);
+        S.eq_word[pos] = Q.L.eq_word; S.eq_count[pos] = Q.L.eq_count;
 #pragma unroll
         for (int i = 0; i < NFF; ++i) {
-            S.eq_ffc[i * C + c] = Q.ffc[i]; S.eq_ffw[i * C + c] = Q.ffw[i];
-            S.eq_snap_ffc[i * C + c] = Q.sffc[i]; S.eq_snap_ffw[i * C + c] = Q.sffw[i];
+            S.eq_ffc[i * C + pos] = Q.ffc[i]; S.eq_ffw[i * C + pos] = Q.ffw[i];
+            S.eq_snap_ffc[i * C + pos] = Q.sffc[i]; S.eq_snap_ffw[i * C + pos] = Q.sffw[i];
         }
 #pragma unroll
         for (int i = 0; i < NFB; ++i) {
-            S.eq_fbc[i * C + c] = Q.fbc[i]; S.eq_fbw[i * C + c] = Q.fbw[i];
-            S.eq_snap_fbc[i * C + c] = Q.sfbc[i]; S.eq_snap_fbw[i * C + c] = Q.sfbw[i];
+            S.eq_fbc[i * C + pos] = Q.fbc[i]; S.eq_fbw[i * C + pos] = Q.fbw[i];
+            S.eq_snap_fbc[i * C + pos] = Q.sfbc[i]; S.eq_snap_fbw[i * C + pos] = Q.sfbw[i];
         }
     } else {
         sym_setprio<sym_prio<NT>(6)>(P);
         Lane L;
         SymFramer F;
         uint8_t *fr_rows;
-        { const State S0 = fresh_state(); lane_load(L, S0, c); fr_rows = S0.fr_msg; }
+        { const State S0 = fresh_state(); lane_load(L, S0, pos); fr_rows = S0.fr_msg; }
         F.st = fr_state(L); F.last = (L.flags & F_LINK_MASK) >> F_LINK_SHIFT;
         F.word = L.fr_word; F.count = L.fr_count; F.invalid = L.fr_invalid; F.len = L.fr_len;
-        uint8_t *const row = fr_rows + (size_t)c * kBurstCap;
+        uint8_t *const row = fr_rows + (size_t)pos * kBurstCap;
         Output O{};
         { const Output Of = fresh_output(); O.n_events = Of.n_events; O.bursts = Of.bursts; O.burst_cap = Of.burst_cap; }
         lds_barrier();
@@ -1596,9 +1588,8 @@
                         const int j = __builtin_ctzll(pend);
                         pend &= pend - 1ull;
                         const uint32_t b = base + k++;
-                        const uint32_t cj = (uint32_t)__builtin_amdgcn_readlane((int)c, j);
                         if (b < O.burst_cap) {
-                            const uint32_t *src = reinterpret_cast<const uint32_t *>(fr_rows + (size_t)cj * kBurstCap);
+                            const uint32_t *src = reinterpret_cast<const uint32_t *>(fr_rows + (size_t)(vwg * kWave + (uint32_t)j) * kBurstCap);
                             uint32_t *dst = reinterpret_cast<uint32_t *>(O.bursts + (size_t)b * kBurstCap);
                             constexpr uint32_t kWords = (uint32_t)kBurstCap / 4u, kPer = (kWords + kWave - 1u) / kWave;
                             uint32_t t[kPer];
@@ -1645,8 +1636,8 @@
         if (gave_up()) return;
         const uint32_t flags_out = (F.st << F_FR_STATE_SHIFT) | (F.last << F_LINK_SHIFT) | (phasebox[lane] & F_TED_PHASE) | (againbox[lane] & F_TICK_AGAIN) | flagbox[lane];
         const State S1 = fresh_state();
-        S1.fr_word[c] = F.word; S1.fr_count[c] = F.count; S1.fr_invalid[c] = F.invalid;
-        S1.fr_len[c] = F.len; S1.flags[c] = flags_out;
+        S1.fr_word[pos] = F.word; S1.fr_count[pos] = F.count; S1.fr_invalid[pos] = F.invalid;
+        S1.fr_len[pos] = F.len; S1.flags[pos] = flags_out;
     }
 }
 
diff --git a/sameold_amd/csrc/same_launch.h b/sameold_amd/csrc/same_launch.h
--- a/sameold_amd/csrc/same_launch.h
+++ b/sameold_amd/csrc/same_launch.h
@@ -45,7 +45,8 @@
 hipError_t launch_reset_columns(const Params &P, const State &S, const uint32_t *cols, uint32_t n, hipStream_t stream);
 hipError_t launch_copy_state_columns(const StateArrayDesc *desc, uint32_t n_desc, uint32_t src_channels,
                                      uint32_t dst_channels, const uint32_t *src_col, uint32_t n_cols, hipStream_t stream,
-                                     uint32_t src_base = 0);
+                                     uint32_t src_base = 0,
+                                     const uint32_t *dst_map = nullptr, const uint32_t *src_map = nullptr);
 hipError_t launch_chunk_final_column(const uint64_t *handover, uint32_t in_channels, ChunkGeom g, uint32_t *final_col,
                                      hipStream_t stream);
 hipError_t launch_chunk_final_column_pc(const uint64_t *handover, const uint32_t *own_start, uint32_t in_channels, uint32_t n_chunks,
@@ -62,6 +63,7 @@
 hipError_t launch_tp_plan(const float *x, const TpPlan &g, float *energy, uint32_t *own_start, uint32_t *row0,
                           uint32_t *nominal, uint32_t *perm, uint32_t *wg_blocks, bool sorted, hipStream_t stream,
                           uint32_t *perm_out = nullptr, uint32_t *wg_blocks_out = nullptr, bool pairs = false);
+hipError_t launch_tp_position_map(const uint32_t *perm, uint32_t *inv, uint32_t columns, hipStream_t stream);
 hipError_t launch_transpose(const float *in, float *out, uint32_t n_channels, uint32_t n_samples,
                             hipStream_t stream);
 hipError_t launch_transpose(const int16_t *in, int16_t *out, uint32_t n_channels, uint32_t n_samples,
diff --git a/sameold_amd/csrc/same_tp_plan.cpp b/sameold_amd/csrc/same_tp_plan.cpp
--- a/sameold_amd/csrc/same_tp_plan.cpp
+++ b/sameold_amd/csrc/same_tp_plan.cpp
@@ -55,10 +55,13 @@
     np.whole_samples = (uint32_t)n; np.in_samples = n_call;
     np.scout_blocks = (uint32_t)(n / kScoutBlock);
     np.energy_floats = (size_t)C * np.scout_blocks;
-    np.pair_groups = cfg.sort_mode == 2 && family == Family::kSym;
-    np.sort_mode = np.pair_groups ? 0 : (cfg.sort_mode >= 0 ? (cfg.sort_mode ? 1 : 0) : (tp_more_than_one_round(columns) ? 1 : 0));
+    const bool regroup = cfg.sort_mode == 3 && family == Family::kSym && !tp_more_than_one_round(columns);
+    const int asked = cfg.sort_mode == 3 ? -1 : cfg.sort_mode;
+    np.pair_groups = regroup || (asked == 2 && family == Family::kSym);
+    np.sort_mode = regroup ? 1 : (np.pair_groups ? 0 : (asked >= 0 ? (asked ? 1 : 0) : (tp_more_than_one_round(columns) ? 1 : 0)));
     np.lpt = np.sort_mode != 0 || np.pair_groups;
-    np.need_hist = np.lpt && family == Family::kSym;
+    np.pos_map = np.lpt && family == Family::kSym;
+    np.need_hist = np.lpt && family == Family::kSym && !regroup;
     np.hist_floats = np.need_hist ? (size_t)columns * kSquelchHist : 0;
     const size_t groups = columns / kWave;
     TpGeomWords &w = np.words;
diff --git a/sameold_amd/csrc/same_tp_plan.h b/sameold_amd/csrc/same_tp_plan.h
--- a/sameold_amd/csrc/same_tp_plan.h
+++ b/sameold_amd/csrc/same_tp_plan.h
@@ -49,6 +49,7 @@
     int sort_mode = 0;
     bool pair_groups = false;
     bool lpt = false;
+    bool pos_map = false;
     bool need_hist = false;
     size_t hist_floats = 0, energy_floats = 0;
     TpGeomWords words;
diff --git a/sameold_amd/receiver.py b/sameold_amd/receiver.py
--- a/sameold_amd/receiver.py
+++ b/sameold_amd/receiver.py
@@ -172,6 +172,7 @@
     sig("same_batch_time_parallel_chunks", u32, vp)
     sig("same_batch_time_parallel_per_channel", C.c_int, vp)
     sig("same_batch_debug_tp_plan", C.c_int, vp, P(TpPlanInfo), vp, C.c_size_t, vp, C.c_size_t, vp, C.c_size_t, vp, C.c_size_t)
+    sig("same_batch_debug_tp_position_map", C.c_int, vp, P(u32), vp, C.c_size_t)
     sig("same_batch_transport_on_device", C.c_int, vp)
     sig("same_batch_set_audio_capture", C.c_int, vp, C.c_size_t)
     sig("same_batch_peek_audio", C.c_int, vp, P(P(AudioChunk)), P(C.c_size_t))
@@ -404,6 +405,14 @@
         out = {name: int(getattr(info, name)) for name, _ in TpPlanInfo._fields_ if name != "reserved"}
         out.update(energy=energy, geom=geom, handover=handover, final_col=final_col)
         return out
+
+    def debug_tp_position_map(self) -> np.ndarray:
+        n = C.c_uint32()
+        _check(self._L.same_batch_debug_tp_position_map(self._h, C.byref(n), C.c_void_p(), 0))
+        inv = np.empty(n.value, np.uint32)
+        if n.value:
+            _check(self._L.same_batch_debug_tp_position_map(self._h, C.byref(n), C.c_void_p(inv.ctypes.data), inv.size))
+        return inv
 
     def set_audio_capture(self, samples_per_launch: int) -> None:
         _check(self._L.same_batch_set_audio_capture(self._h, int(samples_per_launch)))
```

New measurement: 355,800. -24.1%, worse.
